# andyljones/megastep

Hardware: AMD Instinct MI355X
Metric: env-steps/sec (higher is better)
Workload: dtype f32

## Files before the change

include/megastep_hip.h:

```cpp
#ifndef MEGASTEP_HIP_H
#define MEGASTEP_HIP_H

#ifdef __cplusplus
extern "C" {
#endif

#define MS_ABI_VERSION 17

#define MS_OK            0
#define MS_EINVAL       -1
#define MS_EHIP         -2
#define MS_EUNSUPPORTED -3
#define MS_ENODEVICE    -4

typedef struct MsConfig {
    float agent_radius;
    int   res;
    float fov;
    float fps;
} MsConfig;

typedef struct MsScenery {
    int n_envs, n_agents, n_model;
    const float* lights_vals;
    const int*   lights_widths;
    const int*   lights_starts;
    float*       lines_vals;
    const int*   lines_widths;
    const int*   lines_starts;
    const int*   lines_inverse;
    const float* textures_vals;
    const int*   textures_widths;
    const int*   textures_starts;
    const int*   textures_inverse;
    const float* model;
    float*       baked_vals;
    int n_lines_total, n_lights_total, n_texels_total;
    unsigned*    lg_vals;
    const int*   lg_starts;
    const float* lg_geom;
    float        lg_cell;
    int          lg_max_cells;
    unsigned*    lg_list;
    unsigned*    lg_pool;
    int          lg_pool_size;
    float*       lg_pool_rows;
    const int*   env_geom;
    unsigned long long* bake_vis;
    const long long*    bake_vis_starts;
    long long           bake_vis_words;
    const unsigned*       wg_cells;
    const int*            wg_starts;
    const float*          wg_geom;
    float                 wg_cell;
    float                 wg_reach_lo, wg_reach;
    float                 wg_near;
    const unsigned*       wg_pool;
    const long long*      wg_pool_base;
    const float*          wg_near_rows;
    float model_radius;
} MsScenery;

typedef struct MsAgents {
    float* angles;
    float* positions;
    float* angvelocity;
    float* velocity;
    float* headings;
} MsAgents;

typedef struct MsRender {
    int*   indices;
    float* locations;
    float* dots;
    float* distances;
    float* screen;
    int*   workspace;
    float* obs_rgb;
    float* obs_depth;
    int    obs_subsample;
    float  obs_max_depth;
    int*   obs_centre;
    int*       seen_stamp;
    const int* seen_epoch;
    int*       seen_count;
} MsRender;

#define MS_RENDER_WORKSPACE_INTS(N, A, R) (18 + (long long)(N)*(A)*(((R) + 63)/64) + 2*(long long)(N)*(A))

int         ms_abi_version(void);
const char* ms_strerror(int code);
int         ms_last_hip_error(void);
int         ms_device_count(void);

int ms_bake(const MsScenery* scenery, const MsConfig* config, void* hip_stream);

typedef struct MsMovement {
    const long long* actions;
    const float*     table;
    int              n_actions;
    float            keep;
} MsMovement;

typedef struct MsStepExtras {
    unsigned char*   respawn_mask;
    const long long* respawn_choice;
    const float*     spawn_positions;
    const float*     spawn_angles;
    int              n_spawns;
    int              respawn_after;
    int*             lifespans;
    int*             max_lifespans;
    const int*       fresh_max;
    float*           imu;
    float            imu_ang_scale, imu_speed_scale;
} MsStepExtras;

int ms_move_physics(const MsScenery* scenery, const MsAgents* agents, const MsMovement* movement ,
                    float* progress, const MsConfig* config, void* hip_stream);
int ms_physics(const MsScenery* scenery, const MsAgents* agents, float* progress,
               const MsConfig* config, void* hip_stream);
int ms_step_physics(const MsScenery* scenery, const MsAgents* agents, const MsMovement* movement, const MsStepExtras* extras,
                    float* progress, const MsConfig* config, void* hip_stream);

int ms_render(const MsScenery* scenery, const MsAgents* agents, const MsRender* out,
              const MsConfig* config, void* hip_stream);

int ms_step_render(const MsScenery* scenery, const MsAgents* agents, float* progress, const MsRender* out,
                   const MsConfig* config, void* hip_stream);
int ms_move_step_render(const MsScenery* scenery, const MsAgents* agents, const MsMovement* movement, const MsStepExtras* extras,
                        float* progress, const MsRender* out, const MsConfig* config, void* hip_stream);

typedef struct MsDeathmatch {
    const int*      centre;
    const float*    positions;
    const float*    upper;
    float           clearance, hit_damage, tick_damage;
    float*          health;
    float*          damage;
    unsigned char*  dead;
    unsigned char*  reset_out;
    float*          reward;
    float*          health_obs;
    unsigned char*  matchings;
} MsDeathmatch;
int ms_deathmatch_shoot(int n_envs, int n_agents, const MsDeathmatch* dm, void* hip_stream);

typedef struct MsExplorer {
    int*            tally;
    int*            before;
    int*            lengths;
// ... 85 lines not shown
```

megastep_amd/_lib.py:

```python
import ctypes as C
import os
import subprocess
import torch

_HERE = os.path.dirname(os.path.abspath(__file__))
CSRC = os.path.join(_HERE, 'csrc')
LIB_PATH = os.environ.get('MEGASTEP_HIP_LIB') or os.path.join(CSRC, 'libmegastep_hip.so')
ABI_VERSION = 17

_f32p = C.POINTER(C.c_float)
_i32p = C.POINTER(C.c_int)


class MsConfig(C.Structure):
    _fields_ = [('agent_radius', C.c_float), ('res', C.c_int), ('fov', C.c_float), ('fps', C.c_float)]


class MsScenery(C.Structure):
    _fields_ = [
        ('n_envs', C.c_int), ('n_agents', C.c_int), ('n_model', C.c_int),
        ('lights_vals', C.c_void_p), ('lights_widths', C.c_void_p), ('lights_starts', C.c_void_p),
        ('lines_vals', C.c_void_p), ('lines_widths', C.c_void_p), ('lines_starts', C.c_void_p),
        ('lines_inverse', C.c_void_p),
        ('textures_vals', C.c_void_p), ('textures_widths', C.c_void_p), ('textures_starts', C.c_void_p),
        ('textures_inverse', C.c_void_p),
        ('model', C.c_void_p), ('baked_vals', C.c_void_p),
        ('n_lines_total', C.c_int), ('n_lights_total', C.c_int), ('n_texels_total', C.c_int),
        ('lg_vals', C.c_void_p), ('lg_starts', C.c_void_p), ('lg_geom', C.c_void_p), ('lg_cell', C.c_float),
        ('lg_max_cells', C.c_int), ('lg_list', C.c_void_p), ('lg_pool', C.c_void_p), ('lg_pool_size', C.c_int), ('lg_pool_rows', C.c_void_p),
        ('env_geom', C.c_void_p), ('bake_vis', C.c_void_p), ('bake_vis_starts', C.c_void_p), ('bake_vis_words', C.c_longlong),
        ('wg_cells', C.c_void_p), ('wg_starts', C.c_void_p), ('wg_geom', C.c_void_p), ('wg_cell', C.c_float),
        ('wg_reach_lo', C.c_float), ('wg_reach', C.c_float), ('wg_near', C.c_float), ('wg_pool', C.c_void_p), ('wg_pool_base', C.c_void_p), ('wg_near_rows', C.c_void_p),
        ('model_radius', C.c_float)]


class MsWallGridParent(C.Structure):
    _fields_ = [('cells', C.c_void_p), ('starts', C.c_void_p), ('geom', C.c_void_p), ('cell', C.c_float), ('pool', C.c_void_p)]


class MsAgents(C.Structure):
    _fields_ = [('angles', C.c_void_p), ('positions', C.c_void_p), ('angvelocity', C.c_void_p), ('velocity', C.c_void_p),
                ('headings', C.c_void_p)]


class MsMovement(C.Structure):
    _fields_ = [('actions', C.c_void_p), ('table', C.c_void_p), ('n_actions', C.c_int), ('keep', C.c_float)]


class MsStepExtras(C.Structure):
    _fields_ = [('respawn_mask', C.c_void_p), ('respawn_choice', C.c_void_p), ('spawn_positions', C.c_void_p),
                ('spawn_angles', C.c_void_p), ('n_spawns', C.c_int), ('respawn_after', C.c_int),
                ('lifespans', C.c_void_p), ('max_lifespans', C.c_void_p), ('fresh_max', C.c_void_p),
                ('imu', C.c_void_p), ('imu_ang_scale', C.c_float), ('imu_speed_scale', C.c_float)]


class MsRender(C.Structure):
    _fields_ = [('indices', C.c_void_p), ('locations', C.c_void_p), ('dots', C.c_void_p), ('distances', C.c_void_p),
                ('screen', C.c_void_p), ('workspace', C.c_void_p), ('obs_rgb', C.c_void_p), ('obs_depth', C.c_void_p),
                ('obs_subsample', C.c_int), ('obs_max_depth', C.c_float), ('obs_centre', C.c_void_p),
                ('seen_stamp', C.c_void_p), ('seen_epoch', C.c_void_p), ('seen_count', C.c_void_p)]


class MsDeathmatch(C.Structure):
    _fields_ = [('centre', C.c_void_p), ('positions', C.c_void_p), ('upper', C.c_void_p), ('clearance', C.c_float), ('hit_damage', C.c_float),
                ('tick_damage', C.c_float), ('health', C.c_void_p), ('damage', C.c_void_p), ('dead', C.c_void_p), ('reset_out', C.c_void_p),
                ('reward', C.c_void_p), ('health_obs', C.c_void_p), ('matchings', C.c_void_p)]


class MsExplorer(C.Structure):
    _fields_ = [('tally', C.c_void_p), ('before', C.c_void_p), ('lengths', C.c_void_p), ('epoch', C.c_void_p), ('over', C.c_void_p),
                ('slack', C.c_int), ('pixels', C.c_int), ('reset_out', C.c_void_p), ('reward', C.c_void_p), ('potential', C.c_void_p),
                ('length_out', C.c_void_p)]


class MsRaycast(C.Structure):
    _fields_ = [('n_rays', C.c_int), ('origins', C.c_void_p), ('dirs', C.c_void_p), ('near_plane', C.c_float),
                ('indices', C.c_void_p), ('locations', C.c_void_p), ('dots', C.c_void_p), ('distances', C.c_void_p),
                ('agents', C.c_void_p), ('grid_rays', C.c_void_p)]


class MsOverhead(C.Structure):
    _fields_ = [('n_images', C.c_int), ('n_views', C.c_int), ('height', C.c_int), ('width', C.c_int), ('envs', C.c_void_p),
                ('views', C.c_void_p), ('half_width', C.c_float), ('lit', C.c_int), ('background', C.c_float*3),
                ('rgb', C.c_void_p), ('indices', C.c_void_p)]


class MsNavGrid(C.Structure):
    _fields_ = [('n_envs', C.c_int), ('cell', C.c_float), ('clearance', C.c_float), ('geom', C.c_void_p), ('starts', C.c_void_p),
                ('max_framed', C.c_int), ('free_cells', C.c_void_p)]


class MsNavFields(C.Structure):
    _fields_ = [('n_goals', C.c_int), ('goals', C.c_void_p), ('mask', C.c_void_p), ('fields', C.c_void_p), ('passes', C.c_void_p)]


class MsNavQuery(C.Structure):
    _fields_ = [('n_points', C.c_int), ('points', C.c_void_p), ('goal', C.c_void_p), ('fields', C.c_void_p), ('n_goals', C.c_int),
                ('out', C.c_void_p)]


SYMBOLS = ('ms_host_ray_interval_wide', 'ms_debug_ray_groups', 'ms_debug_last_render_groups', 'ms_debug_last_step_fused', 'ms_step_render', 'ms_move_step_render', 'ms_debug_ray_group_tail', 'ms_debug_physics_pack', 'ms_host_render_plan', 'ms_host_render_block', 'ms_host_physics_pack', 'ms_debug_pair_telemetry', 'ms_test_arithmetic', 'ms_abi_version', 'ms_strerror', 'ms_last_hip_error', 'ms_device_count', 'ms_bake', 'ms_physics', 'ms_move_physics',
           'ms_step_physics', 'ms_deathmatch_shoot', 'ms_explorer_books',
           'ms_render', 'ms_raycast', 'ms_camera_rays', 'ms_overhead', 'ms_nav_free', 'ms_nav_fields', 'ms_nav_query', 'ms_debug_overhead_cull', 'ms_host_overhead_keeps', 'ms_host_sincospi', 'ms_host_bake_point_bin', 'ms_host_bake_wall_bins',
           'ms_wallgrid_scan', 'ms_wallgrid_fill', 'ms_host_wall_hidden', 'ms_host_wall_sectors', 'ms_host_wallgrid_cell', 'ms_host_wall_arc',
           'ms_host_wedge_meets', 'ms_host_agents_apart', 'ms_host_wall_beyond_reach', 'ms_host_ray_interval', 'ms_host_fold_hits', 'ms_host_lightgrid_cell', 'ms_host_wall_reach')


def _source_hash():
    import hashlib
    h = hashlib.sha256()
    import glob
    for path in (os.path.join(CSRC, 'megastep_hip.hip'), *sorted(glob.glob(os.path.join(CSRC, 'kernels', '*.h'))),
                 os.path.join(_HERE, '..', 'include', 'megastep_hip.h'), os.path.join(_HERE, '..', 'include', 'megastep_hip_test.h'),
                 os.path.join(CSRC, 'Makefile')):
        with open(path, 'rb') as f:
            h.update(f.read())
    return h.hexdigest()


def build(force=False):
    import fcntl
    stamp = LIB_PATH + '.srchash'
    want = _source_hash()

    def fresh():
        return os.path.exists(LIB_PATH) and os.path.exists(stamp) and open(stamp).read().strip() == want

    if force or not fresh():
        with open(os.path.join(CSRC, '.build.lock'), 'w') as lock:
            fcntl.flock(lock, fcntl.LOCK_EX)
            if force or not fresh():
                import shutil
                hipcc = os.environ.get('HIPCC', '/opt/rocm/bin/hipcc')
                if shutil.which('make') is None or shutil.which(hipcc) is None or not os.access(CSRC, os.W_OK):
                    raise NoToolchain(f'no make / {hipcc} on this host, or {CSRC} is read-only')
                proc = subprocess.run(['make', '-C', CSRC, '-B', 'libmegastep_hip.so'], capture_output=True, text=True)
                if proc.returncode != 0:
                    raise RuntimeError(f'hipcc build of libmegastep_hip.so failed:\n{proc.stdout}\n{proc.stderr}')
    return LIB_PATH


class NoToolchain(OSError):
    """The library cannot be rebuilt here for want of tools (not because its sources do not compile)."""


_lib = None


def lib():
    global _lib
    if _lib is None:
        if not os.environ.get('MEGASTEP_HIP_LIB'):
            try:
                build()
            except NoToolchain as e:
                if not os.path.exists(LIB_PATH):
                    raise
                import warnings
                warnings.warn(f'{LIB_PATH} could not be rebuilt from the sources next to it ({e}); loading it as it is')
        handle = C.CDLL(LIB_PATH)
        missing = [s for s in SYMBOLS if not hasattr(handle, s)]
        if missing:
            raise ImportError(f'{LIB_PATH} does not export {missing}')
        handle.ms_abi_version.restype = C.c_int
        handle.ms_strerror.restype = C.c_char_p
        handle.ms_strerror.argtypes = [C.c_int]
        handle.ms_last_hip_error.restype = C.c_int
        handle.ms_device_count.restype = C.c_int
        handle.ms_bake.argtypes = [C.POINTER(MsScenery), C.POINTER(MsConfig), C.c_void_p]
        handle.ms_physics.argtypes = [C.POINTER(MsScenery), C.POINTER(MsAgents), C.c_void_p, C.POINTER(MsConfig), C.c_void_p]
        handle.ms_move_physics.argtypes = [C.POINTER(MsScenery), C.POINTER(MsAgents), C.POINTER(MsMovement), C.c_void_p,
                                           C.POINTER(MsConfig), C.c_void_p]
        handle.ms_step_physics.argtypes = [C.POINTER(MsScenery), C.POINTER(MsAgents), C.POINTER(MsMovement), C.POINTER(MsStepExtras),
                                           C.c_void_p, C.POINTER(MsConfig), C.c_void_p]
        handle.ms_step_render.argtypes = [C.POINTER(MsScenery), C.POINTER(MsAgents), C.c_void_p, C.POINTER(MsRender), C.POINTER(MsConfig), C.c_void_p]
        handle.ms_step_render.restype = C.c_int
        handle.ms_move_step_render.argtypes = [C.POINTER(MsScenery), C.POINTER(MsAgents), C.POINTER(MsMovement), C.POINTER(MsStepExtras),
                                               C.c_void_p, C.POINTER(MsRender), C.POINTER(MsConfig), C.c_void_p]
        handle.ms_move_step_render.restype = C.c_int
        handle.ms_debug_last_step_fused.argtypes = []
        handle.ms_debug_last_step_fused.restype = C.c_int
        handle.ms_explorer_books.argtypes = [C.c_int, C.POINTER(MsExplorer), C.c_void_p]
        handle.ms_explorer_books.restype = C.c_int
        handle.ms_deathmatch_shoot.argtypes = [C.c_int, C.c_int, C.POINTER(MsDeathmatch), C.c_void_p]
        handle.ms_deathmatch_shoot.restype = C.c_int
        handle.ms_render.argtypes = [C.POINTER(MsScenery), C.POINTER(MsAgents), C.POINTER(MsRender), C.POINTER(MsConfig), C.c_void_p]
        handle.ms_raycast.argtypes = [C.POINTER(MsScenery), C.POINTER(MsAgents), C.POINTER(MsRaycast), C.POINTER(MsConfig), C.c_void_p]
        handle.ms_camera_rays.argtypes = [C.POINTER(MsAgents), C.c_int, C.c_int, C.POINTER(MsConfig), C.c_void_p, C.c_void_p]
        handle.ms_overhead.argtypes = [C.POINTER(MsScenery), C.POINTER(MsAgents), C.POINTER(MsOverhead), C.c_void_p]
        handle.ms_nav_free.argtypes = [C.POINTER(MsScenery), C.POINTER(MsNavGrid), C.c_void_p]
        handle.ms_nav_fields.argtypes = [C.POINTER(MsNavGrid), C.POINTER(MsNavFields), C.c_void_p]
        handle.ms_nav_query.argtypes = [C.POINTER(MsNavGrid), C.POINTER(MsNavQuery), C.c_void_p]
        handle.ms_debug_overhead_cull.argtypes = [C.c_int]
        handle.ms_debug_overhead_cull.restype = C.c_int
        handle.ms_host_overhead_keeps.argtypes = [_f32p, C.c_int, C.c_int, C.c_int, C.c_int, C.c_float, _f32p]
        handle.ms_host_overhead_keeps.restype = C.c_int
        handle.ms_host_sincospi.argtypes = [C.c_float, _f32p, _f32p]
        handle.ms_host_bake_point_bin.argtypes = [C.c_float]*4
        handle.ms_host_bake_point_bin.restype = C.c_int
        handle.ms_host_bake_wall_bins.argtypes = [C.c_float]*6 + [_i32p, _i32p]
        handle.ms_host_bake_wall_bins.restype = None
        handle.ms_wallgrid_scan.argtypes = [C.POINTER(MsScenery), C.POINTER(MsWallGridParent), C.c_void_p, C.c_int, C.c_int, C.c_void_p,
                                            C.c_void_p, C.c_void_p, C.c_void_p]
        handle.ms_wallgrid_fill.argtypes = [C.POINTER(MsScenery), C.c_void_p, C.c_int, C.c_int, C.c_void_p, C.c_void_p, C.c_void_p,
                                            C.c_void_p, C.c_void_p, C.c_void_p]
        handle.ms_host_wall_sectors.argtypes = [C.c_float]*4 + [_f32p, _i32p, _i32p, _f32p, _i32p]
        handle.ms_host_wall_sectors.restype = None
        handle.ms_host_wall_arc.argtypes = [C.c_float]*4 + [_f32p, _i32p, _i32p]
        handle.ms_host_wall_arc.restype = None
        handle.ms_host_wedge_meets.argtypes = [C.c_float]*4 + [C.c_int, C.c_int]
        handle.ms_host_wedge_meets.restype = C.c_int
        handle.ms_host_ray_interval.argtypes = [_f32p, _f32p, C.c_int, C.c_float, C.c_float, C.c_int, _i32p, _i32p]
        handle.ms_host_ray_interval.restype = None
        handle.ms_host_ray_interval_wide.argtypes = [_f32p, _f32p, C.c_int, C.c_float, C.c_float, C.c_int, C.c_int, _i32p, _i32p]
        handle.ms_host_ray_interval_wide.restype = None
        handle.ms_debug_ray_groups.argtypes = [C.c_int]
        handle.ms_debug_ray_groups.restype = C.c_int
        handle.ms_debug_last_render_groups.argtypes = []
        handle.ms_debug_last_render_groups.restype = C.c_int
        handle.ms_debug_ray_group_tail.argtypes = [C.c_float, C.c_int]
        handle.ms_debug_physics_pack.argtypes = [C.c_int]
        handle.ms_debug_physics_pack.restype = C.c_int
        handle.ms_host_render_plan.argtypes = [C.c_int, C.c_int, C.c_int, C.c_int, C.c_int, C.c_float, C.c_int, C.POINTER(C.c_int)]
        handle.ms_host_render_plan.restype = C.c_longlong
        handle.ms_host_render_block.argtypes = [C.c_int, C.c_int, C.c_int, C.c_int, C.c_int, C.c_float, C.c_int, C.c_longlong, C.POINTER(C.c_int)]
        handle.ms_host_render_block.restype = C.c_int
        handle.ms_host_physics_pack.argtypes = [C.c_int, C.c_int, C.c_int, C.c_int]
        handle.ms_host_physics_pack.restype = C.c_int
        handle.ms_debug_ray_group_tail.restype = C.c_int
        handle.ms_debug_pair_telemetry.argtypes = [C.c_int]
        handle.ms_debug_pair_telemetry.restype = C.c_int
        handle.ms_test_arithmetic.argtypes = [C.c_void_p]*7 + [C.c_longlong, C.c_void_p]
        handle.ms_test_arithmetic.restype = C.c_int
        handle.ms_host_fold_hits.argtypes = [_f32p, _i32p, C.c_int, _i32p, _f32p, _i32p]
        handle.ms_host_fold_hits.restype = C.c_int
        handle.ms_host_lightgrid_cell.argtypes = [C.c_void_p, C.c_int, C.c_void_p, C.c_int, C.c_float, C.c_float, C.c_int, C.c_int, C.c_float,
                                                  C.c_int, C.c_void_p, C.c_void_p, C.c_int]
        handle.ms_host_lightgrid_cell.restype = C.c_int
        handle.ms_host_agents_apart.argtypes = [_f32p, _f32p, C.c_float]
        handle.ms_host_agents_apart.restype = C.c_int
        handle.ms_host_wall_beyond_reach.argtypes = [_f32p, _f32p, C.c_float]
        handle.ms_host_wall_beyond_reach.restype = C.c_int
        handle.ms_host_wall_reach.argtypes = [_f32p, C.c_float]
        handle.ms_host_wall_reach.restype = C.c_float
        handle.ms_host_wall_hidden.argtypes = [C.c_float]*4 + [_f32p, _f32p, C.c_float]
        handle.ms_host_wall_hidden.restype = C.c_int
        handle.ms_host_wallgrid_cell.argtypes = [C.c_void_p, C.c_int, C.c_float, C.c_float, C.c_int, C.c_int, C.c_float, C.c_int,
                                                 C.c_float, C.c_float, C.c_float, C.c_void_p, C.c_void_p]
        handle.ms_host_wallgrid_cell.restype = None
        for name in ('ms_bake', 'ms_physics', 'ms_move_physics', 'ms_step_physics', 'ms_render', 'ms_raycast', 'ms_camera_rays', 'ms_overhead', 'ms_nav_free', 'ms_nav_fields', 'ms_nav_query', 'ms_wallgrid_scan', 'ms_wallgrid_fill'):
            getattr(handle, name).restype = C.c_int
        if handle.ms_abi_version() != ABI_VERSION:
            raise ImportError(f'{LIB_PATH} has ABI {handle.ms_abi_version()}, this package needs {ABI_VERSION}; rebuild it')
        _lib = handle
    return _lib


def check(code):
    if code != 0:
        h = lib()
        raise RuntimeError(f'megastep_hip: {h.ms_strerror(code).decode()} (code {code}, hipError {h.ms_last_hip_error()})')


_raw_stream = getattr(torch._C, '_cuda_getCurrentRawStream', None)


def _stream(dev):
    if _raw_stream is not None and dev.index is not None:
        return C.c_void_p(_raw_stream(dev.index))
    return C.c_void_p(torch.cuda.current_stream(dev).cuda_stream)


class _on:

    def __init__(self, dev):
        self._guard = None if dev.index == torch.cuda.current_device() else torch.cuda.device(dev)

    def __enter__(self):
        if self._guard is not None:
            self._guard.__enter__()

    def __exit__(self, *exc):
        if self._guard is not None:
            self._guard.__exit__(*exc)
```

megastep_amd/csrc/kernels/lighting.h:

```cpp
__device__ inline bool light_blocked(P2 I, P2 U, float ax, float ay, float vx, float vy) {
    const P2 V = p2(vx, vy);
    const float UxV = cross(U, V);
    const float ad = fabsf(UxV);
    if (ad < 1.e-3f) return false;
    const P2 PQ = p2(ax, ay) - I;
    const uint32_t sg = f_bits(UxV) & 0x80000000u;
    const float nt = bits_f(f_bits(cross(PQ, U)) ^ sg);
    const float cs = cross(PQ, V);
    const float ns = bits_f(f_bits(cs) ^ sg);
    if (!((nt > 0.f) & (nt < ad) & (ns > 0.f))) return false;
    return div_inrange(cs, UxV) < .999f;
}

struct LightPair { float ax, ay, vx, vy, ix, iy; int light; int pad; };
constexpr int LG_PAIRS = 64;

struct LightScene {
    int n_agents, n_model;
    const float* lights_vals; const int* lights_widths; const int* lights_starts;
    const unsigned* lg_vals; const int* lg_starts; const float* lg_geom; float lg_cell;
    const unsigned* lg_list; const unsigned* lg_pool; const float4* lg_pool_rows;
    unsigned by_m_mul, by_m_sh1, by_m_sh2;
};

__device__ inline float grid_light_intensity(
        const LightScene sc, const MsAgents& ag, const int n, const int lane, const bool dynamic, const int nearest_idx,
        const float cx_l, const float cy_l, const int L, const float4* __restrict__ ln,
        LightPair* s_pair, unsigned* s_shadow, unsigned& telemetry, [[maybe_unused]] unsigned* clk = nullptr) {
#if MS_PROBE
#define LG_CLK(k, v) { asm volatile("" :: "v"(v)); clk[k] = (unsigned)clock64(); }
#else
#define LG_CLK(k, v)
#endif
    const int A = sc.n_agents, AF = sc.n_agents*sc.n_model;
    const int n_lights = sc.lights_widths[n];
    const bool MANY = n_lights > WAVE;
    float acc_in = AMBIENT;
    for (int first_light = 0; ; first_light += WAVE) {
    const int ni = min(WAVE, n_lights - first_light);
    const float* __restrict__ lights = sc.lights_vals + 3*((size_t)sc.lights_starts[n] + first_light);
    const float4 geom = reinterpret_cast<const float4*>(sc.lg_geom)[n];
    float Ix = 0.f, Iy = 0.f, Ii = 0.f;
    if (lane < ni) { Ix = lights[3*lane]; Iy = lights[3*lane + 1]; Ii = lights[3*lane + 2]; }
    int my_target = -1;
    if (dynamic) {
        const unsigned t_ = __umulhi(sc.by_m_mul, (unsigned)nearest_idx);
        my_target = (int)((t_ + (((unsigned)nearest_idx - t_) >> sc.by_m_sh1)) >> sc.by_m_sh2);
    }

    uint4 st = make_uint4(0u, 0u, 0u, 0u);
    uint2 lst = make_uint2(0u, 0u);
    if (!MANY) {
        const float fx = floorf((cx_l - geom.x)/sc.lg_cell), fy = floorf((cy_l - geom.y)/sc.lg_cell);
        const bool inside = dynamic & (fx >= 0.f) & (fx < geom.z) & (fy >= 0.f) & (fy < geom.w);
        const size_t cell_id = (size_t)sc.lg_starts[n] + (inside ? (int)fy*(int)geom.z + (int)fx : 0);
        const uint4 st_ = reinterpret_cast<const uint4*>(sc.lg_vals)[cell_id];
        uint2 lst_ = make_uint2(0u, 0u);
        if (sc.lg_list) lst_ = reinterpret_cast<const uint2*>(sc.lg_list)[cell_id];
        st.x = inside ? st_.x : 0u; st.y = inside ? st_.y : 0u; st.z = inside ? st_.z : 0u; st.w = inside ? st_.w : 0u;
        lst.x = inside ? lst_.x : 0u; lst.y = inside ? lst_.y : 0u;
    }
    LG_CLK(0, st.x + __float_as_uint(Ii))
    const bool shortcut = !MANY && __ballot((lane < ni) & !(Ii >= 0.f)) == 0ull;
    const bool light_ok = ((Ii == 0.f) || ((Ii >= 1.e-12f) && (Ii <= 1.e12f))) && (fabsf(Ix) <= 1.e6f) && (fabsf(Iy) <= 1.e6f);
    const bool point_ok = (fabsf(cx_l) <= 1.e6f) && (fabsf(cy_l) <= 1.e6f);
    const bool nice = __ballot(((lane < ni) && !light_ok) || (dynamic && !point_ok)) == 0ull;
    auto contribution = [&](const float num, const float den) { return nice ? div_inrange(num, den) : num/den; };
    float part = AMBIENT;
    for (unsigned long long rem = MANY ? 0ull : __ballot(dynamic); rem; ) {
        const int j = __ffsll((long long)rem) - 1;
        const unsigned sw[4] = {(unsigned)__builtin_amdgcn_readlane((int)st.x, j), (unsigned)__builtin_amdgcn_readlane((int)st.y, j),
                                (unsigned)__builtin_amdgcn_readlane((int)st.z, j), (unsigned)__builtin_amdgcn_readlane((int)st.w, j)};
        const bool same = dynamic & (st.x == sw[0]) & (st.y == sw[1]) & (st.z == sw[2]) & (st.w == sw[3]);
        rem &= ~__ballot(same);
        #pragma unroll
        for (int k = 0; k < 4; k++) {
            for (unsigned lw = sw[k] & ~(sw[k] >> 1) & 0x55555555u; lw; lw &= lw - 1) {
                const int i = 16*k + ((__ffs((int)lw) - 1) >> 1);
                const float d2 = len2(p2(readlane_f(Ix, i), readlane_f(Iy, i)) - p2(cx_l, cy_l));
                if (same) part += contribution(LUMINANCE*readlane_f(Ii, i), ms_max(d2, 1.f));
            }
        }
    }
    bool has_unk = false;
    {
        const unsigned wd[4] = {st.x, st.y, st.z, st.w};
        #pragma unroll
        for (int k = 0; k < 4; k++) {
            const int nv = min(max(ni - 16*k, 0), 16);
            const unsigned valid = (nv == 16) ? 0x55555555u : (((1u << (2*nv)) - 1u) & 0x55555555u);
            has_unk |= (~(wd[k] | (wd[k] >> 1)) & valid) != 0u;
        }
    }
    LG_CLK(1, part)
    const bool saturated = dynamic & shortcut & (part >= 1.001f);
    const bool need = dynamic & !saturated & has_unk;
    if (!__ballot(need)) return MANY ? acc_in : (saturated ? 1.f : ms_min(part, 1.f));
    telemetry = 0x80000000u | (unsigned)__popcll(__ballot(need)) | ((unsigned)min(ni, 63) << 25);

    auto status = [&](int i) {
        const unsigned wd = (i < 16) ? st.x : (i < 32) ? st.y : (i < 48) ? st.z : st.w;
        return (wd >> (2*(i & 15))) & 3u;
    };
    unsigned long long shadow = 0ull;
    const bool sweep = need & (lst.y == 0u);
    const int n_cd = (need & !sweep) ? (int)(lst.y & 0x7fffffffu) : 0;
    telemetry |= (unsigned)__popcll(__ballot(sweep)) << 7;
    if (__ballot(n_cd > 0)) {
        s_shadow[2*lane] = 0u; s_shadow[2*lane + 1] = 0u;
// ... 153 lines not shown
```

megastep_amd/csrc/kernels/overhead.h:

```cpp
constexpr int OV_TILE = 16;
constexpr int OV_CHUNK = 1024;
static_assert(OV_TILE*OV_TILE == WG, "one pixel per lane");
static_assert(OV_CHUNK % WG == 0 && OV_CHUNK >= 2*WG, "a window of WG lines must fit after a partly filled list");

struct OvArgs {
    const int* envs;
    const float* views;
    float* rgb;
    int* indices;
    long long block0;
    int n_views, height, width, tiles_x, tiles_y;
    float half_width, h2;
    float bg_r, bg_g, bg_b;
    int lit, with_agents, cull;
};

struct OvBox { float x0, y0, x1, y1, mag; bool finite; };

__host__ __device__ inline OvBox ov_footprint(const float g0, const float g1, const float g2, const float g3, const float g4,
                                              const float g5, const int i0, const int j0, const int i1, const int j1) {
    const float ua = (float)j0 + .5f, ub = (float)j1 + .5f, wa = (float)i0 + .5f, wb = (float)i1 + .5f;
    const float xs[4] = {(g0*ua + g1*wa) + g2, (g0*ub + g1*wa) + g2, (g0*ua + g1*wb) + g2, (g0*ub + g1*wb) + g2};
    const float ys[4] = {(g3*ua + g4*wa) + g5, (g3*ub + g4*wa) + g5, (g3*ua + g4*wb) + g5, (g3*ub + g4*wb) + g5};
    OvBox b{xs[0], ys[0], xs[0], ys[0], 0.f, true};
    for (int c = 0; c < 4; c++) {
        b.finite = b.finite && isfinite(xs[c]) && isfinite(ys[c]);
        b.x0 = fminf(b.x0, xs[c]); b.x1 = fmaxf(b.x1, xs[c]);
        b.y0 = fminf(b.y0, ys[c]); b.y1 = fmaxf(b.y1, ys[c]);
    }
    const float sx = 1e-5f*((fabsf(g0)*ub + fabsf(g1)*wb) + fabsf(g2));
    const float sy = 1e-5f*((fabsf(g3)*ub + fabsf(g4)*wb) + fabsf(g5));
    b.finite = b.finite && isfinite(sx) && isfinite(sy);
    b.x0 -= sx; b.x1 += sx; b.y0 -= sy; b.y1 += sy;
    b.mag = fmaxf(fmaxf(fabsf(b.x0), fabsf(b.x1)), fmaxf(fabsf(b.y0), fabsf(b.y1)));
    return b;
}

__host__ __device__ inline bool ov_keeps(const OvBox& b, const float h, const float4 L) {
    if (!b.finite) return true;
    const float mag = fmaxf(fmaxf(fabsf(L.x), fabsf(L.y)), fmaxf(fabsf(L.z), fabsf(L.w)));
    const float r = h + 1e-5f*(h + mag + b.mag);
    const float x0 = b.x0 - r, x1 = b.x1 + r, y0 = b.y0 - r, y1 = b.y1 + r;
    if ((fmaxf(L.x, L.z) < x0) || (fminf(L.x, L.z) > x1) || (fmaxf(L.y, L.w) < y0) || (fminf(L.y, L.w) > y1)) return false;
    const float vx = L.z - L.x, vy = L.w - L.y;
    const float cx = .5f*(x0 + x1), cy = .5f*(y0 + y1), ex = .5f*(x1 - x0), ey = .5f*(y1 - y0);
    const float qx = cx - L.x, qy = cy - L.y;
    const float sep = fabsf(vx*qy - vy*qx);
    const float reach = ex*fabsf(vy) + ey*fabsf(vx);
    const float tol = 1e-5f*(fabsf(vx) + fabsf(vy))*(fabsf(qx) + fabsf(qy) + ex + ey + fabsf(vx) + fabsf(vy));
    return !(sep > reach + tol);
}

struct OvBest { float d2; int idx; float t; };

__device__ inline void ov_fold(const float x, const float y, const float4 L, const int l, const float h2, OvBest& b) {
    const float vx = L.z - L.x, vy = L.w - L.y, px = x - L.x, py = y - L.y;
    const float vv = vx*vx + vy*vy;
    float t = vv > 0.f ? (px*vx + py*vy)/vv : 0.f;
    t = t < 0.f ? 0.f : (t > 1.f ? 1.f : t);
    const float dx = px - t*vx, dy = py - t*vy;
    const float d2 = dx*dx + dy*dy;
    if ((d2 <= h2) & ((d2 < b.d2) | ((d2 == b.d2) & (l < b.idx)))) { b.d2 = d2; b.idx = l; b.t = t; }
}

__global__ __launch_bounds__(WG) void overhead_kernel(const MsScenery sc, const MsAgents ag, const OvArgs a) {
    __shared__ float4 s_rows[OV_CHUNK];
    __shared__ int s_idx[OV_CHUNK];
    __shared__ int s_wave[WAVES];
    const int tid = threadIdx.x, lane = tid % WAVE, wave = tid / WAVE;
    const long long blk = a.block0 + blockIdx.x;
    const int tiles = a.tiles_x*a.tiles_y;
    const long long kv = blk / tiles;
    const int tile = (int)(blk - kv*tiles);
    const int k = (int)(kv / a.n_views);
    const int ty = tile / a.tiles_x, tx = tile - ty*a.tiles_x;
    const int i0 = ty*OV_TILE, j0 = tx*OV_TILE;
    const int i = i0 + tid / OV_TILE, j = j0 + tid % OV_TILE;
    const bool live = (i < a.height) & (j < a.width);
    const long long hw = (long long)a.height*a.width;
    const long long at = kv*hw + (long long)i*a.width + j;
    const int e = __builtin_amdgcn_readfirstlane(a.envs ? a.envs[k] : k);

    OvBest best{INFINITY, INT_MAX, 0.f};
    int base = 0, AF = 0;
    if ((e >= 0) & (e < sc.n_envs)) {
        const float* const g = a.views + kv*6;
        const float g0 = g[0], g1 = g[1], g2 = g[2], g3 = g[3], g4 = g[4], g5 = g[5];
        const float u = (float)j + .5f, w = (float)i + .5f;
        const float x = (g0*u + g1*w) + g2, y = (g3*u + g4*w) + g5;
        const OvBox box = ov_footprint(g0, g1, g2, g3, g4, g5, i0, j0, min(i0 + OV_TILE - 1, a.height - 1),
                                       min(j0 + OV_TILE - 1, a.width - 1));
        const int L = sc.lines_widths[e];
        base = sc.lines_starts[e];
        const int A = sc.n_agents, M = sc.n_model;
        AF = A*M;
        const float4* const rows = reinterpret_cast<const float4*>(sc.lines_vals) + base;
        int count = 0;
        for (int l0 = 0; l0 < L; l0 += WG) {
            const int l = l0 + tid;
            bool keep = false;
            float4 row = make_float4(0.f, 0.f, 0.f, 0.f);
            if (l < L) {
                if (a.with_agents && l < AF) {
                    const int agent = l / M;
                    float s, c;
                    sincospi_f(ag.angles[e*A + agent]/180.f, s, c);
                    const float2 p = reinterpret_cast<const float2*>(ag.positions)[e*A + agent];
                    row = drawn_row(s, c, p.x, p.y, reinterpret_cast<const float4*>(sc.model)[l - agent*M]);
                } else {
                    row = rows[l];
                }
                keep = !a.cull || ov_keeps(box, a.half_width, row);
            }
            const unsigned long long m = __ballot(keep);
            if (lane == 0) s_wave[wave] = (int)__popcll(m);
            __syncthreads();
            int off = count, total = 0;
            for (int q = 0; q < WAVES; q++) {
                const int c = s_wave[q];
                off += q < wave ? c : 0;
                total += c;
            }
            off += (int)__popcll(m & ((1ull << lane) - 1ull));
            if (keep) { s_rows[off] = row; s_idx[off] = l; }
            count += total;
            __syncthreads();
            if (count > OV_CHUNK - WG || l0 + WG >= L) {
                for (int q = 0; q < count; q++) ov_fold(x, y, s_rows[q], s_idx[q], a.h2, best);
                count = 0;
                __syncthreads();
            }
        }
    }

    if (!live) return;
    float r = a.bg_r, gr = a.bg_g, bl = a.bg_b;
    int idx = -1;
    if (best.idx != INT_MAX) {
        idx = best.idx;
        r = gr = bl = 0.f;
        const int gl = base + idx;
        const int tw = a.rgb ? sc.textures_widths[gl] : 0;
        if (tw > 0) {
            const int q = min((int)(best.t*(float)tw), tw - 1);
            const long long tex = (long long)sc.textures_starts[gl] + q;
            r = sc.textures_vals[3*tex]; gr = sc.textures_vals[3*tex + 1]; bl = sc.textures_vals[3*tex + 2];
            if (a.lit && idx >= AF) {
                const float bk = sc.baked_vals[tex];
// ... 11 lines not shown
```

megastep_amd/csrc/kernels/physics.h:

```cpp
constexpr int PHYS_AHEAD = 4;
constexpr int PHYS_FEW = 4;
constexpr int PHYS_PAIRS = (PHYS_FEW + 1)*WAVE;

__device__ inline void spawn_pose(const MsStepExtras& ex, const int i, float2& p, float& ang) {
    const long long c = min(max(ex.respawn_choice[i], 0ll), (long long)ex.n_spawns - 1);
    p = reinterpret_cast<const float2*>(ex.spawn_positions)[(size_t)i*ex.n_spawns + c];
    ang = ex.spawn_angles[(size_t)i*ex.n_spawns + c];
}
__device__ inline int lifespan_tick(const MsStepExtras& ex, const int i, bool& reset) {
    const int life = ex.lifespans[i] + 1;
    reset = reset | (life >= ex.max_lifespans[i]);
    return reset ? 0 : life;
}
__device__ inline void move_velocity(const float keep, const float ang, const float dx, const float dy, const float dw, float2& v, float& w) {
    const float a_ = 0.017453292519943295f*ang;
    const float s_ = sinf(a_), c_ = cosf(a_);
    const float gx = c_*dx - s_*dy, gy = s_*dx + c_*dy;
    if (keep == 0.f) { w = dw; v = make_float2(gx, gy); }
    else { w = keep*w + dw; v = make_float2(keep*v.x + gx, keep*v.y + gy); }
}
__device__ inline int near_count(const uint4 hdr, const float reach, const float reach_lo) {
    return (int)((reach <= reach_lo) ? (hdr.w & 0xffffu) : (hdr.w >> 16));
}
__device__ inline bool integrate(const float x, const float fps, float2& p, float& ang, float2& v, float& w) {
    p.x = p.x + x*v.x/fps;
    p.y = p.y + x*v.y/fps;
    ang = normalize_degrees(ang + x*w/fps);
    const bool stopped = x < 1;
    if (stopped) { v = make_float2(0.f, 0.f); w = 0.f; }
    return stopped;
}
__device__ inline float3 imu_reading(const MsStepExtras& ex, const float ang, const float2 v, const float w) {
    const float a_ = 0.017453292519943295f*ang;
    const float s_ = sinf(a_), c_ = cosf(a_);
    return make_float3(w*ex.imu_ang_scale, (c_*v.x + s_*v.y)*ex.imu_speed_scale, (-s_*v.x + c_*v.y)*ex.imu_speed_scale);
}

template <int MOVE, int EXTRA, int PACK = 0>
__global__ __launch_bounds__(WAVE) void physics_kernel(
        const MsScenery sc, const MsAgents ag, float* __restrict__ progress,
        const float agent_radius, const float fps, const MsMovement mv, const MsStepExtras ex, const int pack_envs, const Divisor by_a) {
    PROBE_INIT
    extern __shared__ float4 s_dyn[];
    __shared__ float4 s_wall[PHYS_PAIRS];
    __shared__ int s_tag[PHYS_PAIRS];
    const int A1 = sc.n_agents, AF = sc.n_agents*sc.n_model;
    const int lane = threadIdx.x;
    const int n = PACK ? blockIdx.x*pack_envs : blockIdx.x;
    const int E = PACK ? min(pack_envs, sc.n_envs - n) : 1;
    const int A = PACK ? A1*E : A1;
    const int nA = n*A1;
    [[maybe_unused]] const int lane_env = PACK ? min(div_by(lane, by_a), E - 1) : 0;
    float4* s_task = s_dyn;
    float4* s_box = s_task + A;
    float* s_reach2 = reinterpret_cast<float*>(s_box + A);
    unsigned* s_prog = reinterpret_cast<unsigned*>(s_reach2 + A);
    const float2* pos2 = reinterpret_cast<const float2*>(ag.positions);
    const float2* vel2 = reinterpret_cast<const float2*>(ag.velocity);

    const int L = sc.lines_widths[n];
    const float4* __restrict__ ln = reinterpret_cast<const float4*>(sc.lines_vals) + sc.lines_starts[n];
    const LineRows rows(ln, L);
    const bool gridded = sc.wg_cells != nullptr;
    const float4 wg_geom_n = reinterpret_cast<const float4*>(sc.wg_geom)[n + lane_env];
    const int wg_start_n = sc.wg_starts[n + lane_env];
    float4 w[PHYS_AHEAD];
    #pragma unroll
    for (int k = 0; k < PHYS_AHEAD; k++) w[k] = make_float4(0.f, 0.f, 0.f, 0.f);
    if (!gridded) {
        #pragma unroll
        for (int k = 0; k < PHYS_AHEAD; k++) w[k] = rows.chunk(lane, AF + k*WAVE);
    }
    float2 my_p, my_v;
    float my_w, my_ang;
    my_p = make_float2(0.f, 0.f); my_v = make_float2(0.f, 0.f); my_w = 0.f; my_ang = 0.f;
    if (lane < A) { my_p = pos2[nA + lane]; my_v = vel2[nA + lane]; my_w = ag.angvelocity[nA + lane]; my_ang = ag.angles[nA + lane]; }

    if constexpr (EXTRA == 1) {
        for (int t = lane; t < A; t += WAVE) {
            const int i = nA + t;
            bool reset = ex.respawn_mask && ex.respawn_mask[i];
            if (ex.lifespans) {
                ex.lifespans[i] = lifespan_tick(ex, i, reset);
                if (reset) ex.max_lifespans[i] = ex.fresh_max[i];
                if (ex.respawn_mask) ex.respawn_mask[i] = reset ? 1 : 0;
            }
            if (reset && ex.spawn_positions && !ex.respawn_after) {
                float2 p; float ang;
                spawn_pose(ex, i, p, ang);
                if (t == lane) { my_p = p; my_ang = ang; my_v = make_float2(0.f, 0.f); my_w = 0.f; }
                reinterpret_cast<float2*>(ag.positions)[i] = p;
                ag.angles[i] = ang;
                reinterpret_cast<float2*>(ag.velocity)[i] = make_float2(0.f, 0.f);
                ag.angvelocity[i] = 0.f;
            }
        }
    }
    if constexpr (MOVE == 1) {
        const bool small_table = 3*mv.n_actions <= WAVE;
        const float tab = mv.table[min(lane, 3*mv.n_actions - 1)];
        auto moved = [&](const int i, const float ang, float2& v, float& w, const float dx, const float dy, const float dw) {
            move_velocity(mv.keep, ang, dx, dy, dw, v, w);
            ag.angvelocity[i] = w;
            reinterpret_cast<float2*>(ag.velocity)[i] = v;
        };
        {
            const long long act = min(max(mv.actions[nA + min(lane, A - 1)], 0ll), (long long)mv.n_actions - 1);
            float dx, dy, dw;
            if (small_table) { dx = __shfl(tab, 3*(int)act, WAVE); dy = __shfl(tab, 3*(int)act + 1, WAVE); dw = __shfl(tab, 3*(int)act + 2, WAVE); }
            else { dx = mv.table[3*act]; dy = mv.table[3*act + 1]; dw = mv.table[3*act + 2]; }
            if (lane < A) moved(nA + lane, my_ang, my_v, my_w, dx, dy, dw);
        }
        for (int t = lane + WAVE; t < A; t += WAVE) {
            float2 v = vel2[nA + t];
            float w = ag.angvelocity[nA + t];
            const long long act = min(max(mv.actions[nA + t], 0ll), (long long)mv.n_actions - 1);
            moved(nA + t, ag.angles[nA + t], v, w, mv.table[3*act], mv.table[3*act + 1], mv.table[3*act + 2]);
        }
    }
    float4 my_box = make_float4(INFINITY, INFINITY, -INFINITY, -INFINITY);
    float my_reach = 0.f;
    for (int t = lane; t < A; t += WAVE) {
        const float2 pp = (t == lane) ? my_p : pos2[nA + t], mm = (t == lane) ? my_v : vel2[nA + t];
        const P2 p0 = p2(pp.x, pp.y);
        const P2 v0 = p2(mm.x, mm.y)/fps;
        const float reach = wall_reach(p0, v0, agent_radius);
        s_reach2[t] = reach_squared(reach);
        const float4 box = make_float4(p0.x - reach, p0.y - reach, p0.x + reach, p0.y + reach);
        if (t == lane) { my_box = box; my_reach = (reach == reach) ? reach : INFINITY; }
        s_box[t] = box;
        s_task[t] = make_float4(p0.x, p0.y, v0.x, v0.y);
// ... 200 lines not shown
```

megastep_amd/csrc/kernels/raycast.h:

```cpp

struct RayFold { float s; int idx; float t, vx, vy; };

__device__ inline void ray_fold(const P2 p, const P2 ru, const float near_s, const float4 L, const int l, RayFold& f) {
    const P2 v = p2(L.z - L.x, L.w - L.y);
    const P2 pq = p2(L.x, L.y) - p;
    const float d = cross(ru, v), nt = cross(pq, ru);
    const float ad = fabsf(d);
    const float ntp = __uint_as_float(__float_as_uint(nt) ^ (__float_as_uint(d) & 0x80000000u));
    if ((ad >= 1.e-3f) & (ntp <= ad) & (ntp >= -1e-30f*ad)) {
        const Isect q = intersect(p, ru, p2(L.x, L.y), v);
        const bool hit = (0 <= q.t) & (q.t <= 1);
        const bool better = (near_s < q.s) & (q.s < f.s - 1.e-4f);
        if (hit & better) { f.s = q.s; f.idx = l; f.t = q.t; f.vx = v.x; f.vy = v.y; }
    }
}

__global__ __launch_bounds__(WG) void raycast_kernel(const MsScenery sc, const MsAgents ag, const MsRaycast q, const int with_agents,
                                                     const int gridded, const int n_total) {
    const int i_raw = blockIdx.x*WG + threadIdx.x;
    const bool live = i_raw < n_total;
    const int i = live ? i_raw : n_total - 1;
    const int n = i / q.n_rays;
    const float2 o = reinterpret_cast<const float2*>(q.origins)[i];
    const float2 d = reinterpret_cast<const float2*>(q.dirs)[i];
    const P2 p = p2(o.x, o.y), ru = p2(d.x, d.y);
    const float rlen = len(ru);
    const float near_s = q.near_plane/rlen;
    const int A = sc.n_agents, M = sc.n_model, AF = A*M;
    RayFold f{INFINITY, -1, NAN, 0.f, 0.f};
    auto fold_agents = [&](const int e) {
        for (int a = 0; a < A; a++) {
            float s, c;
            sincospi_f(ag.angles[e*A + a]/180.f, s, c);
            const float2 pa = reinterpret_cast<const float2*>(ag.positions)[e*A + a];
            for (int m = 0; m < M; m++)
                ray_fold(p, ru, near_s, drawn_row(s, c, pa.x, pa.y, reinterpret_cast<const float4*>(sc.model)[m]), a*M + m, f);
        }
    };
    const int n_w = __builtin_amdgcn_readfirstlane(n);
    const bool one_env = __ballot(n != n_w) == 0ull;

    if (one_env) {
        const int L = sc.lines_widths[n_w];
        const float4* const rows = reinterpret_cast<const float4*>(sc.lines_vals) + sc.lines_starts[n_w];
        if (with_agents) fold_agents(n_w);
        bool listed = false;
        int cell = -1;
        if (gridded) {
            bool inside;
            const int c = wg_cell_at(reinterpret_cast<const float4*>(sc.wg_geom)[n_w], sc.wg_cell, p.x, p.y, inside);
            const float ru2 = len2(ru);
            listed = inside & (ru2 >= 1.f) & (ru2 <= WG_MAX_RU2);
            cell = listed ? sc.wg_starts[n_w] + c : -1;
        }
        unsigned long long pending = __ballot(listed);
        int walk = 0;
        for (unsigned long long todo = pending; todo && walk <= L - AF;) {
            const int cell_w = __builtin_amdgcn_readlane(cell, __ffsll((long long)todo) - 1);
            walk += (int)reinterpret_cast<const uint4*>(sc.wg_cells)[cell_w].y;
            todo &= ~__ballot(cell == cell_w);
        }
        if (walk > L - AF) pending = 0ull;
        bool done = false;
        while (pending) {
            const int cell_w = __builtin_amdgcn_readlane(cell, __ffsll((long long)pending) - 1);
            const uint4 hdr = reinterpret_cast<const uint4*>(sc.wg_cells)[cell_w];
            const int count = (int)hdr.y;
            const bool mine = cell == cell_w;
            pending &= ~__ballot(mine);
            if (mine) {
                int wa8, wb8;
                const float pa = pseudo_angle(ru.x, ru.y);
                wg_wedge(pa, pa, wa8, wb8);
                const unsigned* const vis = sc.wg_pool + sc.wg_pool_base[n_w] + hdr.x;
                for (int k = 0; k < count; k++) {
                    const unsigned e = vis[k];
                    const int l = AF + (int)(e & 0xffffu);
                    if (wg_arcs_meet((int)((e >> 16) & 255u), (int)(e >> 24), wa8, wb8) & (l < L)) ray_fold(p, ru, near_s, rows[l], l, f);
                }
                done = true;
            }
        }
        if (__ballot(!done))
            for (int l = AF; l < L; l++) {
                const float4 row = rows[l];
                if (!done) ray_fold(p, ru, near_s, row, l, f);
            }
        if (q.grid_rays) {
            const unsigned long long took = __ballot(live & done);
            if (took && (int)threadIdx.x % WAVE == __ffsll((long long)__ballot(1)) - 1) atomicAdd(q.grid_rays, (int)__popcll(took));
        }
    } else {
        const int L = sc.lines_widths[n];
        const float4* const rows = reinterpret_cast<const float4*>(sc.lines_vals) + sc.lines_starts[n];
        if (with_agents) fold_agents(n);
        for (int l = AF; l < L; l++) ray_fold(p, ru, near_s, rows[l], l, f);
    }

    if (!live) return;
    float dt = NAN;
// ... 24 lines not shown
```

megastep_amd/csrc/kernels/render.h:

```cpp
constexpr int PAIRS = 128;

struct Cand { float pqx, pqy, vx, vy; };

__device__ __attribute__((noinline)) float2 sincospi_called(const float x) {
    float s_, c_;
    sincospi_f(x, s_, c_);
    return make_float2(s_, c_);
}

__device__ inline float4 drawn_row(const float s, const float c, const float px, const float py, const float4 mdl) {
    float4 w;
    w.x = c*mdl.x - s*mdl.y + px; w.y = s*mdl.x + c*mdl.y + py;
    w.z = c*mdl.z - s*mdl.w + px; w.w = s*mdl.z + c*mdl.w + py;
    return w;
}
__device__ inline void camera_ray(const float cs, const float sn, const int r, const float Rf, const float half_screen,
                                  const float inv_res, float& rx, float& ry) {
    const float num = (Rf - 2*(float)r - 1)*half_screen;
    const float uy = inv_res != 0.f ? num*inv_res : div_inrange(num, Rf);
    rx = cs*1.f - sn*uy; ry = sn*1.f + cs*uy;
}
__host__ inline float camera_inv_res(const int R, const float half_screen) {
    return ((R & (R - 1)) == 0 && half_screen > 1e-3f) ? 1.f/(float)R : 0.f;
}

__device__ __attribute__((noinline)) float4 drawn_line_of(const float* angles, const float* positions, const float* model,
                                                          const int n_agents, const int M, const int n, const int l) {
    const int a = l / M, m = l - a*M;
    float s, c;
    sincospi_f(angles[n*n_agents + a]/180.f, s, c);
    const float2 p = reinterpret_cast<const float2*>(positions)[n*n_agents + a];
    return drawn_row(s, c, p.x, p.y, reinterpret_cast<const float4*>(model)[m]);
}
__device__ inline float4 drawn_line(const MsScenery& sc, const MsAgents& ag, int n, int l) {
    return drawn_line_of(ag.angles, ag.positions, sc.model, sc.n_agents, sc.n_model, n, l);
}

struct Filt { int l, r; float lw, rw; };
__device__ inline Filt tex_filter(float x, int w) {
    Filt f;
    const float y = ms_min(x*(w + 1), (float)(w - 1));
    f.l = (int)ms_max(y - 1, 0.f);
    f.r = (int)ms_min(y, (float)(w - 1));
    const float ld = fabsf(y - (f.l + 1)) + 1.e-3f;
    const float rd = fabsf(y - (f.r + 1)) + 1.e-3f;
    const float den = ld + rd, r_den = rcp_refined(den);
    f.lw = div_by_refined(rd, den, r_den);
    f.rw = div_by_refined(ld, den, r_den);
    return f;
}

__device__ inline float sqrt_normal(const float x) {
    const float s = __builtin_amdgcn_sqrtf(x);
    const float dn = bits_f(f_bits(s) - 1u), up = bits_f(f_bits(s) + 1u);
    const float r_dn = __builtin_fmaf(-dn, s, x), r_up = __builtin_fmaf(-up, s, x);
    float r = (r_dn <= 0.f) ? dn : s;
    r = (r_up > 0.f) ? up : r;
    return r;
}

__device__ __attribute__((noinline)) float sqrtf_called(const float x) { return sqrtf(x); }
__device__ inline float sqrt_any(const float x) {
    float r = sqrt_normal(x);
    if (__builtin_expect(!(x >= 1.e-30f) && x != 0.f, 0) || __builtin_expect(!(x <= 1.e30f), 0)) r = sqrtf_called(x);
    return r;
}

struct RenderConsts {
    float x_clip, c_b;
    Divisor by_f, by_g, by_m;
    Divisor by_f1, by_g1;
    int envs_lo, envs_rem, tail;
    int skip_own;
    float inv_res;
    int telemetry;
    int ws_headings;
};
struct RenderConstsStep : RenderConsts {
    float* progress;
    float fps;
    const unsigned* wg_cells_physics;
    MsMovement mv;
    MsStepExtras ex;
};
enum { OUT_INDICES = 1, OUT_LOCATIONS = 2, OUT_DOTS = 4, OUT_DISTANCES = 8, OUT_SCREEN = 16, OUT_RGB = 32, OUT_DEPTH = 64, OUT_CENTRE = 128,
       OUT_SEEN = 256 };
__global__ __launch_bounds__(WG) void arithmetic_test_kernel(const float* __restrict__ n, const float* __restrict__ d, float* __restrict__ q_inrange,
                                                             float* __restrict__ q_ieee, const float* __restrict__ x, float* __restrict__ r_any,
                                                             float* __restrict__ r_ieee, const long long count) {
    const long long i = (long long)blockIdx.x*WG + threadIdx.x;
    if (i >= count) return;
    if (q_inrange) q_inrange[i] = div_by_refined(n[i], d[i], rcp_refined(d[i]));
    if (q_ieee) q_ieee[i] = n[i]/d[i];
    if (r_any) r_any[i] = sqrt_any(x[i]);
    if (r_ieee) r_ieee[i] = sqrtf(x[i]);
}

__host__ __device__ inline bool render_block(const int b, const int n_blocks, const int A, const int R, const int ng, const RenderConsts& rc,
                                             int& n, int& a, int& r0, int& span, int& fan) {
    const int xcd = b & 7, ix = b >> 3;
    fan = b;
    if (ng == 1) {
        const int q8 = n_blocks >> 3, r8 = n_blocks & 7;
        fan = xcd*q8 + (xcd < r8 ? xcd : r8) + ix;
        const int G = (R + WAVE - 1)/WAVE, F = A*G;
        n = div_by(fan, rc.by_f); const int rem = fan - n*F; a = div_by(rem, rc.by_g); r0 = (rem - a*G)*WAVE; span = WAVE;
        return true;
    }
    const int NR = ng*WAVE;
    const int e_x = rc.envs_lo + (xcd < rc.envs_rem ? 1 : 0), first_x = xcd*rc.envs_lo + (xcd < rc.envs_rem ? xcd : rc.envs_rem);
    const int t_x = rc.tail < e_x ? rc.tail : e_x;
    const int Gw = (R + NR - 1)/NR, w_x = (e_x - t_x)*A*Gw;
    const bool single = ix >= w_x;
    const int f = single ? ix - w_x : ix;
    const int G = single ? (R + WAVE - 1)/WAVE : Gw, F = A*G;
    const Divisor df = Divisor{single ? rc.by_f1.mul : rc.by_f.mul, single ? rc.by_f1.sh1 : rc.by_f.sh1, single ? rc.by_f1.sh2 : rc.by_f.sh2};
    const Divisor dg = Divisor{single ? rc.by_g1.mul : rc.by_g.mul, single ? rc.by_g1.sh1 : rc.by_g.sh1, single ? rc.by_g1.sh2 : rc.by_g.sh2};
    const int nn = div_by(f, df), rem = f - nn*F;
    if (nn >= (single ? t_x : e_x - t_x)) return false;
    a = div_by(rem, dg);
    n = first_x + (single ? e_x - t_x : 0) + nn;
    span = single ? WAVE : NR;
    r0 = (rem - a*G)*span;
    return true;
}

__global__ __launch_bounds__(WG) void render_prep_kernel(const MsAgents ag, int* __restrict__ workspace,
                                                         const int n_agents_total, const int headings_at) {
    const int i = blockIdx.x*WG + threadIdx.x;
    if (i == 0) { workspace[0] = 0; workspace[1] = 0; workspace[2] = 0; workspace[3] = 0; workspace[4] = 0; }
    if (i < n_agents_total) {
        float s, c;
        sincospi_f(ag.angles[i]/180.f, s, c);
        reinterpret_cast<float2*>(workspace + headings_at)[i] = make_float2(s, c);
    }
}


struct RenderArgs { MsScenery sc; MsAgents ag; MsRender out; float agent_radius, half_screen; int R, n_fans; RenderConsts rc; };
static_assert(offsetof(RenderArgs, ag) == sizeof(MsScenery) && offsetof(RenderArgs, n_fans) + 4 == offsetof(RenderArgs, rc),
              "RenderArgs must mirror render_kernel's parameters");
typedef const RenderArgs __attribute__((address_space(4)))* LateArgs;
__device__ inline LateArgs late_args() {
    LateArgs p = (LateArgs)__builtin_amdgcn_kernarg_segment_ptr();
    asm volatile("" : "+s"(p));
    return p;
}

__host__ inline uint32_t host_f_bits(const float f) { uint32_t u; memcpy(&u, &f, 4); return u; }
__host__ inline float host_bits_f(const uint32_t u) { float f; memcpy(&f, &u, 4); return f; }
__host__ inline unsigned long long slot_min(unsigned long long* slot, const unsigned long long key) {
    const unsigned long long old = *slot;
    if (key < old) *slot = key;
    return old;
}
__host__ inline unsigned long long hit_key(const float sv, const int line) { return ((unsigned long long)host_f_bits(sv) << 32) | (unsigned)line; }
__host__ inline bool hit_loser_matters(const unsigned long long key, const float sv, const unsigned long long old, unsigned long long& lose1) {
    const unsigned oh = (unsigned)(old >> 32);
    if (oh == 0xffffffffu) return false;
    const bool won = key < old;
    const float so = host_bits_f(oh);
    const float front = won ? sv : so, back = won ? so : sv;
    lose1 = won ? old : key;
    return back < front + 4.e-4f;
}
__host__ inline bool hit_resolve(const unsigned long long best, const unsigned long long second, const unsigned long long third,
                                 float& nearest_s, int& nearest_idx) {
    bool ambiguous = false;
    if (best != ~0ull) {
        const float s1 = host_bits_f((uint32_t)(best >> 32)), s2 = host_bits_f((uint32_t)(second >> 32)), s3 = host_bits_f((uint32_t)(third >> 32));
        const int i1 = (int)(uint32_t)best, i2 = (int)(uint32_t)second;
        nearest_s = s1;
        nearest_idx = i1;
        if ((second != ~0ull) && !(s1 < s2 - 1.e-4f)) {
            if ((third == ~0ull) || (s2 < s3 - 1.e-4f)) {
                const bool first_is_1 = i1 < i2;
                const float sa = first_is_1 ? s1 : s2, sb = first_is_1 ? s2 : s1;
                const int ia = first_is_1 ? i1 : i2, ib = first_is_1 ? i2 : i1;
                const bool b_wins = sb < sa - 1.e-4f;
                nearest_s = b_wins ? sb : sa;
                nearest_idx = b_wins ? ib : ia;
            } else {
                ambiguous = true;
            }
        }
    }
    return ambiguous;
}

__host__ __device__ inline float rcp_approx(const float x) {
#if defined(__HIP_DEVICE_COMPILE__)
    return __builtin_amdgcn_rcpf(x);
#else
    return 1.f/x;
#endif
}
__host__ __device__ inline void agent_frame(const float cs, const float sn, const float pqx, const float pqy, const float dbx, const float dby,
                                            float& xa, float& ya, float& xb, float& yb) {
    xa = __builtin_fmaf(cs, pqx, sn*pqy); ya = __builtin_fmaf(cs, pqy, -(sn*pqx));
    xb = __builtin_fmaf(cs, dbx, sn*dby); yb = __builtin_fmaf(cs, dby, -(sn*dbx));
}
__host__ __device__ inline void ray_interval(float xa, float ya, float xb, float yb, const bool live, const float x_clip,
                                    const float c_a, const float c_b, const float g0, const float last_local, int& lo, int& len,
                                    const float n_rays = 64.f) {
    const bool fa = xa >= x_clip, fb = xb >= x_clip;
    const bool inc = fa | fb;
    const float ia = fa ? ya*rcp_approx(xa) : 0.f, ib = fb ? yb*rcp_approx(xb) : 0.f;
    const float fra = __builtin_fmaf(-ia, c_b, c_a), frb = __builtin_fmaf(-ib, c_b, c_a);
    const float marg = __builtin_fmaf(1e-4f, fabsf(fra) + fabsf(frb), 0.05f);
    const float edge = (xa*yb - ya*xb > 0.f) ? -INFINITY : INFINITY;
    const float ra = fa ? fra : -edge, rb = fb ? frb : edge;
    const float flo = fminf(fmaxf(fminf(ra, rb) - (marg + g0), 0.f), n_rays);
    const float fhi = fmaxf(fminf(fmaxf(ra, rb) + (marg - g0), last_local), -1.f);
    lo = (int)ceilf(flo);
    const int n_ = (int)floorf(fhi) - lo + 1;
    len = (live & inc) ? (n_ > 0 ? n_ : 0) : 0;
}

#ifndef MS_WAVES
#define MS_WAVES 6
#endif
#ifndef MS_AHEAD
#define MS_AHEAD 1
#endif
#ifndef MS_VCAP
#define MS_VCAP 128
#endif
#ifndef MS_VCAP_WIDE
#define MS_VCAP_WIDE 110
#endif
#ifndef MS_WAVES_WIDE
#define MS_WAVES_WIDE 6
#endif
template <int OBS, int SHADE = 1, int NG = 1, int STEP = 0>
__global__ __launch_bounds__(WAVE) __attribute__((amdgpu_waves_per_eu(NG > 1 ? MS_WAVES_WIDE : MS_WAVES, NG > 1 ? MS_WAVES_WIDE : MS_WAVES))) void render_kernel(
        const MsScenery sc, const MsAgents ag, const MsRender out,
        const float agent_radius, const float half_screen, const int R, const int n_fans,
        const std::conditional_t<STEP == 1, RenderConstsStep, RenderConsts> rc) {
    static_assert(STEP == 0 || NG == 1, "the fused step: one group of rays");
    PROBE_INIT
    static_assert(NG == 1 || NG == 2 || NG == 4, "one, two or four ray groups per wave");
    [[maybe_unused]] constexpr int NR = WAVE*NG;
    constexpr int VCAP = NG == 1 ? MS_VCAP : MS_VCAP_WIDE;
    constexpr int O_EPI = NG > 1 ? 24*VCAP + 256 : 0;
    constexpr int LDS_PER_WAVE = NG == 1 ? 24*VCAP + 3072 : O_EPI + 2816 + 6*VCAP;
    __shared__ __attribute__((aligned(16))) unsigned char s_raw[LDS_PER_WAVE];

    int lane = threadIdx.x;
#define LANE_AFRESH asm volatile("" : "+v"(lane))
    Cand* const s_cand_w = reinterpret_cast<Cand*>(&s_raw[0]);
    float* const s_screen_w = reinterpret_cast<float*>(&s_raw[O_EPI]);

    const int b = blockIdx.x;
    [[maybe_unused]] int fan = b;
    const int A = sc.n_agents, AF = sc.n_agents*sc.n_model;
    int n, a, r0, span;
    if (!render_block(b, n_fans, A, R, NG, rc, n, a, r0, span, fan)) return;
    const int r = r0 + lane;
    const int r_last = min(r0 + span - 1, R - 1);
    [[maybe_unused]] const int n_live = r_last - r0 + 1;

    const int L = sc.lines_widths[n];
    const int base = sc.lines_starts[n];
    const float4 wg_geom_n = reinterpret_cast<const float4*>(sc.wg_geom)[n];
    const int wg_start_n = sc.wg_starts[n];
    const long long wg_pool_base_n = sc.wg_pool_base[n];
    float4* __restrict__ ln = reinterpret_cast<float4*>(sc.lines_vals) + base;
    const LineRows rows(ln, L);
    float ag_s = 0.f, ag_c = 0.f;
    float2 ag_p = make_float2(0.f, 0.f);
    auto load_agents = [&]() {
    ag_s = 0.f; ag_c = 0.f; ag_p = make_float2(0.f, 0.f);
    const int lane_a = n*A + min(lane, A - 1);
    if (ag.headings) {
        const float4 h = reinterpret_cast<const float4*>(ag.headings)[lane_a];
        const float angle = ag.angles[lane_a];
        const float2 p_ = reinterpret_cast<const float2*>(ag.positions)[lane_a];
        if (lane < A) {
            ag_s = h.y; ag_c = h.z; ag_p = p_;
            if (f_bits(h.x) != f_bits(angle)) { const float2 sc_ = sincospi_called(angle/180.f); ag_s = sc_.x; ag_c = sc_.y; }
        }
    } else if (lane < A) {
        if (out.workspace) {
            const float2 sc_ = reinterpret_cast<const float2*>(out.workspace + rc.ws_headings)[n*A + lane];
            ag_s = sc_.x; ag_c = sc_.y;
        } else {
            const float2 sc_ = sincospi_called(ag.angles[n*A + lane]/180.f);
            ag_s = sc_.x; ag_c = sc_.y;
        }
        ag_p = reinterpret_cast<const float2*>(ag.positions)[n*A + lane];
    }
    };
    if constexpr (STEP == 1) {
        float2 p_ = reinterpret_cast<const float2*>(ag.positions)[n], v_ = reinterpret_cast<const float2*>(ag.velocity)[n];
        float w_ = ag.angvelocity[n], ang_ = ag.angles[n];
        const MsStepExtras& ex = rc.ex;
        bool respawn_now = false;
        float2 spawn_p = make_float2(0.f, 0.f);
        float spawn_ang = 0.f;
        if (ex.respawn_mask || ex.lifespans) {
            bool reset = ex.respawn_mask && ex.respawn_mask[n];
            if (ex.lifespans) {
                const int life = lifespan_tick(ex, n, reset);
                const int fresh = ex.fresh_max[n];
                __builtin_amdgcn_wave_barrier();
                if (lane == 0) {
                    if (reset) ex.max_lifespans[n] = fresh;
                    ex.lifespans[n] = life;
                    if (ex.respawn_mask) ex.respawn_mask[n] = reset ? 1 : 0;
                }
            }
            if (reset && ex.spawn_positions) {
                spawn_pose(ex, n, spawn_p, spawn_ang);
                respawn_now = true;
                if (!ex.respawn_after) {
                    p_ = spawn_p; ang_ = spawn_ang; v_ = make_float2(0.f, 0.f); w_ = 0.f;
                    if (lane == 0) {
                        reinterpret_cast<float2*>(ag.positions)[n] = p_;
                        ag.angles[n] = ang_;
                        reinterpret_cast<float2*>(ag.velocity)[n] = v_;
                        ag.angvelocity[n] = 0.f;
                    }
                }
            }
        }
        if (rc.mv.actions) {
            const long long act = min(max(rc.mv.actions[n], 0ll), (long long)rc.mv.n_actions - 1);
            move_velocity(rc.mv.keep, ang_, rc.mv.table[3*act], rc.mv.table[3*act + 1], rc.mv.table[3*act + 2], v_, w_);
            if (lane == 0) {
                ag.angvelocity[n] = w_;
                reinterpret_cast<float2*>(ag.velocity)[n] = v_;
            }
        }
        const P2 p0 = p2(p_.x, p_.y);
        const P2 v0 = p2(v_.x, v_.y)/rc.fps;
        const float reach = wall_reach(p0, v0, agent_radius);
        const float reach2 = reach_squared(reach);
        const float my_reach = (reach == reach) ? reach : INFINITY;
        const float4 tk = make_float4(p0.x, p0.y, v0.x, v0.y);
        bool listed_p = false;
// ... 39 lines not shown
            }
            rc.progress[n] = x;
        }
        if (ex.imu) {
            const float3 m = imu_reading(ex, ang_, v_, w_);
            if (lane == 0) {
                ex.imu[3*n] = m.x;
                ex.imu[3*n + 1] = m.y;
                ex.imu[3*n + 2] = m.z;
            }
        }
        ag_s = hsc.x; ag_c = hsc.y; ag_p = p_;
    } else {
        load_agents();
    }
    constexpr int AHEAD = MS_AHEAD;

    const float4 mdl_draw = reinterpret_cast<const float4*>(sc.model)[min(lane, sc.n_model - 1)];
    const float4 mdl_first = reinterpret_cast<const float4*>(sc.model)[lane - div_by(lane, rc.by_m)*sc.n_model];
    auto agent_line_m = [&](const int l_, const bool have_row, const float4 row) {
        const int l = min(max(l_, 0), AF - 1);
        if (A > WAVE) return drawn_line(sc, ag, n, l);
        const int la = div_by(l, rc.by_m);
        const float s_ = __shfl(ag_s, la, WAVE), c_ = __shfl(ag_c, la, WAVE);
        const float px_ = __shfl(ag_p.x, la, WAVE), py_ = __shfl(ag_p.y, la, WAVE);
        float4 mdl = row;
        if (!have_row) mdl = reinterpret_cast<const float4*>(sc.model)[l - la*sc.n_model];
        return drawn_row(s_, c_, px_, py_, mdl);
    };
    auto agent_line = [&](const int l_) { return agent_line_m(l_, false, make_float4(0.f, 0.f, 0.f, 0.f)); };
    float sn, cs;
    float2 pp;
    if (A <= WAVE) {
        sn = readlane_f(ag_s, a); cs = readlane_f(ag_c, a);
        pp = make_float2(readlane_f(ag_p.x, a), readlane_f(ag_p.y, a));
    } else {
        const float2 sc_ = sincospi_called(ag.angles[n*A + a]/180.f);
        sn = sc_.x; cs = sc_.y;
        pp = reinterpret_cast<const float2*>(ag.positions)[n*A + a];
    }
    PROBE_AT(1, pp.x)
    unsigned wg_first = 0u;
    int wg_count = -1;
    if (sc.wg_cells) {
        bool inside;
        const int cell_id = __builtin_amdgcn_readfirstlane(wg_start_n + wg_cell_at(wg_geom_n, sc.wg_cell, pp.x, pp.y, inside));
        const uint4 hdr = reinterpret_cast<const uint4*>(sc.wg_cells)[cell_id];
        wg_first = inside ? hdr.x : 0u;
        wg_count = inside ? (int)hdr.y : -1;
        if constexpr (NG > 1) {
            wg_first = (unsigned)__builtin_amdgcn_readfirstlane((int)wg_first);
            wg_count = __builtin_amdgcn_readfirstlane(wg_count);
        }
    }
    if (r0 == 0) {
        for (int m0 = 0; m0 < sc.n_model; m0 += WAVE) {
            const float4 w = agent_line_m(a*sc.n_model + m0 + lane, m0 == 0, mdl_draw);
            if (m0 + lane < sc.n_model) ln[a*sc.n_model + m0 + lane] = w;
        }
    }
    const float Rf = (float)R;
    auto ray_len = [&](const float rx_, const float ry_) {
        return sqrt_normal(rx_*rx_ + ry_*ry_);
    };
    auto ray_of = [&](const int r_, float& rx_, float& ry_, float& rlen_, float& near_) {
        camera_ray(cs, sn, r_, Rf, half_screen, rc.inv_res, rx_, ry_);
        rlen_ = ray_len(rx_, ry_);
        near_ = div_inrange(agent_radius, rlen_);
    };
    float rx, ry, rlen, near;
    ray_of(r, rx, ry, rlen, near);

    const float c_a = 0.5f*(Rf - 1.f), c_b = rc.c_b;
    const float x_clip = rc.x_clip;
    const float g0 = (float)r0;

    constexpr bool COLOUR = SHADE != 0;
    static_assert(COLOUR || OBS == 1, "without colour `screen` is NULL: the OBS instantiation");
    static_assert(OBS != 2 || (COLOUR && STEP == 0), "no per-ray planes at all: a colour instantiation");
    constexpr bool PLANES = OBS != 2;
    constexpr bool MASKED = !COLOUR || (OBS >= 1 && NG == 1);
    [[maybe_unused]] const int out_mask_ = MASKED ? (out.obs_subsample >> 8) : 0;
#define MS_WANTED(BIT, PTR) (MASKED ? ((out_mask_ & (BIT)) != 0) : ((PTR) != nullptr))
    auto winner_of = [&](const int nearest_idx, float4& hw_mem, int& tex_w, int& tstart) {
        const LateArgs late = late_args();
        const bool want_texel_row = COLOUR || (OBS && MS_WANTED(OUT_SEEN, late->out.seen_stamp));
        const bool want_line = want_texel_row || MS_WANTED(OUT_LOCATIONS, late->out.locations) || MS_WANTED(OUT_DOTS, late->out.dots);
        const int row = min(max(nearest_idx, 0), max(L - 1, 0));
        hw_mem = make_float4(0.f, 0.f, 0.f, 0.f); tex_w = 1; tstart = 0;
        if (want_line) hw_mem = rows.row(row);
        if (want_texel_row) {
            const int* const l_tex_widths = late->sc.textures_widths;
            const int* const l_tex_starts = late->sc.textures_starts;
            tex_w = l_tex_widths[base + row]; tstart = l_tex_starts[base + row];
        }
    };
    auto finish_group = [&](const int q, const int r, const float rx, const float ry, const float rlen,
                            const float nearest_s, const int nearest_idx, const float4 hw_mem, const int tex_w, const int tstart) {
    const LateArgs late = late_args();
    const bool want_texel_row = COLOUR || (OBS && MS_WANTED(OUT_SEEN, late->out.seen_stamp));
    const bool want_line = want_texel_row || MS_WANTED(OUT_LOCATIONS, late->out.locations) || MS_WANTED(OUT_DOTS, late->out.dots);
    float loc = NAN, dt = NAN;
    float4 hw = make_float4(0.f, 0.f, 0.f, 0.f);
    if (want_line) {
        float4 aw = make_float4(0.f, 0.f, 0.f, 0.f);
        if (__ballot((nearest_idx >= 0) & (nearest_idx < AF))) aw = agent_line(nearest_idx);
        if (nearest_idx >= 0) {
            hw = (nearest_idx < AF) ? aw : hw_mem;
            const float vx = hw.z - hw.x, vy = hw.w - hw.y;
            const float d = rx*vy - ry*vx;
            const float pqx = hw.x - pp.x, pqy = hw.y - pp.y;
            loc = div_inrange(pqx*ry - pqy*rx, d);
            const float dtop = rx*vx + ry*vy;
            const float dbot = rlen*sqrt_any(vx*vx + vy*vy);
            dt = div_inrange(dtop, dbot + 1.e-6f);
        }
    }
    [[maybe_unused]] const size_t o = ((size_t)n*A + a)*R + r;
    const float dist = nearest_s*rlen;
    if constexpr (PLANES) {
        if (!MASKED || (out_mask_ & (OUT_INDICES | OUT_LOCATIONS | OUT_DOTS | OUT_DISTANCES))) {
            int* const o_indices = late->out.indices;
            float* const o_locations = late->out.locations;
            float* const o_dots = late->out.dots;
            float* const o_distances = late->out.distances;
            if (r < R) {
                if (!OBS || MS_WANTED(OUT_INDICES, o_indices)) __builtin_nontemporal_store(nearest_idx, &o_indices[o]);
                if (!OBS || MS_WANTED(OUT_LOCATIONS, o_locations)) __builtin_nontemporal_store(loc, &o_locations[o]);
                if (!OBS || MS_WANTED(OUT_DOTS, o_dots)) __builtin_nontemporal_store(dt, &o_dots[o]);
                if (!OBS || MS_WANTED(OUT_DISTANCES, o_distances)) __builtin_nontemporal_store(dist, &o_distances[o]);
            }
        }
    }

    const bool is_hit = (nearest_idx >= 0) & (r < R);
    float s0 = 0.f, s1 = 0.f, s2 = 0.f;
    [[maybe_unused]] Filt f = Filt{0, 0, 0.f, 0.f};
    [[maybe_unused]] float intensity = 0.f;
    [[maybe_unused]] float tl0 = 0.f, tl1 = 0.f, tl2 = 0.f, tr0 = 0.f, tr1 = 0.f, tr2 = 0.f;
    if constexpr (COLOUR) {
        const float* const l_tex_vals = late->sc.textures_vals;
        const float* const l_baked = late->sc.baked_vals;
        const bool dynamic = is_hit & (nearest_idx < AF);
        [[maybe_unused]] unsigned light_telemetry = 0x80000000u;
        if (__ballot(dynamic)) {
            if (sc.lg_vals) {
                __builtin_amdgcn_fence(__ATOMIC_RELEASE, "wavefront");
                __builtin_amdgcn_wave_barrier();
                const float cx_l = hw.x*(1 - loc) + hw.z*loc, cy_l = hw.y*(1 - loc) + hw.w*loc;
                const LightScene scl{sc.n_agents, sc.n_model, late->sc.lights_vals, late->sc.lights_widths, late->sc.lights_starts,
                                     late->sc.lg_vals, late->sc.lg_starts, late->sc.lg_geom, late->sc.lg_cell,
                                     late->sc.lg_list, late->sc.lg_pool, reinterpret_cast<const float4*>(late->sc.lg_pool_rows),
                                     rc.by_m.mul, rc.by_m.sh1, rc.by_m.sh2};
#if MS_PROBE
                unsigned lclk[2] = {0u, 0u};
                PROBE_VAL(14, (unsigned)clock64())
                intensity = grid_light_intensity(scl, ag, n, lane, dynamic, nearest_idx, cx_l, cy_l, L, ln,
                    reinterpret_cast<LightPair*>(&s_raw[O_EPI]), reinterpret_cast<unsigned*>(&s_raw[O_EPI + 2048]), light_telemetry, lclk);
                PROBE_VAL(12, lclk[0]) PROBE_VAL(13, lclk[1]) PROBE_VAL(11, (unsigned)clock64())
#else
                intensity = grid_light_intensity(scl, ag, n, lane, dynamic, nearest_idx, cx_l, cy_l, L, ln,
                    reinterpret_cast<LightPair*>(&s_raw[O_EPI]), reinterpret_cast<unsigned*>(&s_raw[O_EPI + 2048]), light_telemetry);
#endif
                PROBE_VAL(2, light_telemetry)
            } else if constexpr (NG == 1) {
                if (out.workspace && lane == 0) out.workspace[16 + atomicAdd(&out.workspace[0], 1)] = fan;
            }
        }
        PROBE_AT(5, tex_w)
        f = tex_filter(is_hit ? loc : 0.f, tex_w);
        const float bk_l = l_baked[tstart + f.l], bk_r = l_baked[tstart + f.r];
        const float* __restrict__ tl = l_tex_vals + 3*(size_t)(tstart + f.l);
        const float* __restrict__ tr = l_tex_vals + 3*(size_t)(tstart + f.r);
        tl0 = tl[0]; tl1 = tl[1]; tl2 = tl[2]; tr0 = tr[0]; tr1 = tr[1]; tr2 = tr[2];
        if (is_hit & !dynamic) intensity = f.lw*bk_l + f.rw*bk_r;
    }
    if constexpr (OBS >= 1) {
        if (MS_WANTED(OUT_SEEN, late->out.seen_stamp)) {
            bool fresh = false, fresh_last = false;
            const int last_env = sc.n_envs - 1;
            if (is_hit) {
                const float wf = (float)tex_w;
                const int along = (int)ms_min(floorf(wf*loc), wf - 1);
                const int epoch = late->out.seen_epoch[n];
                if (late->out.seen_stamp[tstart + along] != epoch)
                    fresh = atomicExch(&late->out.seen_stamp[tstart + along], epoch) != epoch;
            } else if ((r < R) & (sc.n_texels_total > 0)) {
                const int last = sc.n_texels_total - 1;
                const int epoch = late->out.seen_epoch[last_env];
                if (late->out.seen_stamp[last] != epoch)
                    fresh_last = atomicExch(&late->out.seen_stamp[last], epoch) != epoch;
            }
            const unsigned long long fm = __ballot(fresh);
            if (fm && lane == 0) atomicAdd(&late->out.seen_count[n], __popcll(fm));
            if (__ballot(fresh_last) && lane == 0) atomicAdd(&late->out.seen_count[last_env], 1);
        }
        if (MS_WANTED(OUT_CENTRE, late->out.obs_centre)) {
            const int sub = MASKED ? (late->out.obs_subsample & 0xff) : late->out.obs_subsample, sh = __builtin_ctz((unsigned)sub), W = R >> sh;
            const int r1 = (((W >> 1) - 1) << sh) + (sub >> 1), r2 = ((W >> 1) << sh) + (sub >> 1);
            if ((r == r1) | (r == r2)) {
                int seen = -1;
                if ((nearest_idx >= 0) & (nearest_idx < AF)) seen = div_by(nearest_idx, rc.by_m);
                late->out.obs_centre[((size_t)n*A + a)*2 + (r == r2 ? 1 : 0)] = seen;
            }
        }
    }

    if constexpr (COLOUR) {
        PROBE_AT(6, tl0)
        if (is_hit) {
            const float dn = 1 - dt*dt;
            s0 = dn*intensity*(f.lw*tl0 + f.rw*tr0);
            s1 = dn*intensity*(f.lw*tl1 + f.rw*tr1);
            s2 = dn*intensity*(f.lw*tl2 + f.rw*tr2);
        }
        if constexpr (PLANES) {
        float* const o_screen = late->out.screen;
        if (!OBS || MS_WANTED(OUT_SCREEN, o_screen)) {
            s_screen_w[3*lane] = s0; s_screen_w[3*lane + 1] = s1; s_screen_w[3*lane + 2] = s2;
            __builtin_amdgcn_fence(__ATOMIC_RELEASE, "wavefront");
            __builtin_amdgcn_wave_barrier();
            __builtin_amdgcn_fence(__ATOMIC_ACQUIRE, "wavefront");
            const int nfl = 3*min(n_live - q*WAVE, WAVE);
            float* __restrict__ scr = o_screen + 3*(((size_t)n*A + a)*R + r0 + q*WAVE);
            #pragma unroll
            for (int k = 0; k < 3; k++) {
                const int j = lane + k*WAVE;
                if (j < nfl) __builtin_nontemporal_store(s_screen_w[j], &scr[j]);
            }
        }
        }
    }
    if (OBS && ((COLOUR && MS_WANTED(OUT_RGB, late->out.obs_rgb)) || MS_WANTED(OUT_DEPTH, late->out.obs_depth))) {
        const int sub = MASKED ? (late->out.obs_subsample & 0xff) : late->out.obs_subsample;
        float p0 = s0, p1 = s1, p2 = s2;
        float pd = 1.f - ms_min(ms_max((dist - agent_radius)*late->out.obs_max_depth, 0.f), 1.f);
        auto quad_xor = [](const float v, auto ctrl) {
            return __int_as_float(__builtin_amdgcn_mov_dpp(__float_as_int(v), decltype(ctrl)::value, 0xf, 0xf, true));
        };
        constexpr std::integral_constant<int, 0xB1> XOR1{};
        constexpr std::integral_constant<int, 0x4E> XOR2{};
        if (sub > 1) {
            if constexpr (COLOUR) { p0 += quad_xor(p0, XOR1); p1 += quad_xor(p1, XOR1); p2 += quad_xor(p2, XOR1); }
            pd += quad_xor(pd, XOR1);
        }
        if (sub > 2) {
            if constexpr (COLOUR) { p0 += quad_xor(p0, XOR2); p1 += quad_xor(p1, XOR2); p2 += quad_xor(p2, XOR2); }
            pd += quad_xor(pd, XOR2);
        }
        for (int o2 = 4; o2 < sub; o2 <<= 1) {
            if constexpr (COLOUR) {
                p0 += __shfl_xor(p0, o2, WAVE); p1 += __shfl_xor(p1, o2, WAVE); p2 += __shfl_xor(p2, o2, WAVE);
            }
            pd += __shfl_xor(pd, o2, WAVE);
        }
        if (((lane & (sub - 1)) == 0) & (r < R)) {
            const int sh = __builtin_ctz((unsigned)sub);
            const float inv = bits_f((uint32_t)(127 - sh) << 23);
// ... 149 lines not shown
        int raw_pos = 0, q_len = 0, al_left = AL;
        int q_first = 0;
        for (;;) {
            while ((raw_pos < n_raw) & (q_len <= Q_CAP - WAVE)) {
                const unsigned e = e_next[0];
                e_next[0] = e_next[1];
                e_next[1] = raw(raw_pos + 2*WAVE);
                const int k = raw_pos + lane;
                const int idx = listed ? (int)(e & 0xffffu) : k;
                const bool keep = (k < n_raw) & (!listed | wg_arcs_meet((int)((e >> 16) & 255u), (int)(e >> 24), wa8, wb8));
                const unsigned long long km = __ballot(keep);
                if (keep) s_queue_w[q_len + (int)__builtin_amdgcn_mbcnt_hi((unsigned)(km >> 32), __builtin_amdgcn_mbcnt_lo((unsigned)km, 0u))] = (unsigned short)idx;
                q_len += __popcll(km);
                raw_pos += WAVE;
            }
            __builtin_amdgcn_fence(__ATOMIC_RELEASE, "wavefront");
            __builtin_amdgcn_wave_barrier();
            __builtin_amdgcn_fence(__ATOMIC_ACQUIRE, "wavefront");
            const int al0 = AL - al_left;
            const int n_al = min(al_left, AHEAD*WAVE);
            const int n_items = n_al + min(q_len, AHEAD*WAVE - n_al);
            const int q_used = n_items - n_al;
            int l_it[AHEAD];
            float4 w_it[AHEAD];
            #pragma unroll
            for (int kk = 0; kk < AHEAD; kk++) {
                const int i = kk*WAVE + lane;
                const int ai = al0 + i;
                const int q_at = min(max(i - n_al, 0), Q_CAP - 1);
                const int qe = listed ? (int)s_queue_w[q_at] : q_first + q_at;
                l_it[kk] = (i < n_al) ? ai + (ai >= own0 ? own : 0) : AF + qe;
                w_it[kk] = rows.load(l_it[kk]*16, 0);
            }
            PROBE_VAL(2, 0)
            PROBE_AT(3, w_it[0].x)
            #pragma unroll
            for (int kk = 0; kk < AHEAD; kk++) {
                if (kk*WAVE >= n_items) continue;
                admit_fn(w_it[kk], l_it[kk], kk*WAVE + lane < n_items, kk*WAVE < n_al, al0 + kk*WAVE == 0);
            }
            al_left -= n_al;
            __builtin_amdgcn_wave_barrier();
            if (q_used < q_len) {
                unsigned short keep_[Q_CAP/WAVE];
                #pragma unroll
                for (int j = 0; j < Q_CAP/WAVE; j++) keep_[j] = s_queue_w[min(q_used + j*WAVE + lane, Q_CAP - 1)];
                __builtin_amdgcn_wave_barrier();
                #pragma unroll
                for (int j = 0; j < Q_CAP/WAVE; j++) if (j*WAVE + lane < q_len - q_used) s_queue_w[j*WAVE + lane] = keep_[j];
            }
            q_len -= q_used;
            q_first += q_used;
            if (((raw_pos >= n_raw) & (q_len == 0) & (al_left == 0)) || stop_fn()) break;
        }
    };
    if constexpr (NG == 1) {
        walk(pa_last, pa_first, admit, [] { return false; });
        if (n_pairs) drain();
    }
    __builtin_amdgcn_fence(__ATOMIC_ACQUIRE, "wavefront");
    bool list_whole = true;
    auto resolve_group = [&](const int q, const float rx, const float ry, const float near, float& nearest_s, int& nearest_idx) {
        const unsigned long long best = s_best_w[lane], second = s_second_w[lane], third = s_third_w[lane];
        bool ambiguous = false;
        if (best != ~0ull) {
            const float s1 = bits_f((uint32_t)(best >> 32)), s2 = bits_f((uint32_t)(second >> 32)), s3 = bits_f((uint32_t)(third >> 32));
            const int i1 = (int)(uint32_t)best, i2 = (int)(uint32_t)second;
            nearest_s = s1;
            nearest_idx = i1;
            if ((second != ~0ull) && !(s1 < s2 - 1.e-4f)) {
                if ((third == ~0ull) || (s2 < s3 - 1.e-4f)) {
                    const bool first_is_1 = i1 < i2;
                    const float sa = first_is_1 ? s1 : s2, sb = first_is_1 ? s2 : s1;
                    const int ia = first_is_1 ? i1 : i2, ib = first_is_1 ? i2 : i1;
                    const bool b_wins = sb < sa - 1.e-4f;
                    nearest_s = b_wins ? sb : sa;
                    nearest_idx = b_wins ? ib : ia;
                } else {
                    ambiguous = true;
                }
            }
        }
        const unsigned long long amb = __ballot(ambiguous);
        PROBE_VAL(11, n_pairs_total) PROBE_VAL(12, n_drains == 1 ? list_n : -1) PROBE_VAL(13, __popcll(amb))
#if MS_PROBE
        const unsigned t_fold0 = (unsigned)clock64();
        PROBE_VAL(15, t_fold0)
#endif
        if (out.workspace && lane == 0 && q == 0 && rc.telemetry) {
            atomicAdd(&out.workspace[3], n_pairs_total); atomicAdd(&out.workspace[4], n_windows);
        }
        if (amb && out.workspace && lane == 0) {
            atomicAdd(&out.workspace[1], __popcll(amb));
            if (__popcll(amb) > 6) atomicAdd(&out.workspace[2], 1);
        }
        if (amb && (NG == 1 ? n_drains == 1 : list_whole)) {
            const int rounds = (list_n + WAVE - 1)/WAVE;
            if (2*(int)__popcll(amb)*rounds <= list_n + 16) {
                float x = INFINITY;
                int xi = -1;
                for (int k0 = 0; k0 < list_n; k0 += WAVE) {
                    const int k = min(k0 + lane, list_n - 1);
                    const Cand cd = s_cand_w[k];
                    const int line = s_info_w[k].y;
                    const float cpv = cd.pqx*cd.vy - cd.pqy*cd.vx;
                    for (unsigned long long todo = amb; todo; todo &= todo - 1) {
                        const int jr = __ffsll((long long)todo) - 1;
                        const float jrx = readlane_f(rx, jr), jry = readlane_f(ry, jr), jnear = readlane_f(near, jr);
                        const float d = jrx*cd.vy - jry*cd.vx;
                        const float nt = cd.pqx*jry - cd.pqy*jrx;
                        const float ad = fabsf(d);
                        const float ntp = bits_f(f_bits(nt) ^ (f_bits(d) & 0x80000000u));
                        bool valid = false;
                        float sv = 0.f;
                        if ((k0 + lane < list_n) & (ad >= 1.e-3f) & (ntp >= 0.f) & (ntp <= ad)) {
                            sv = div_inrange(cpv, d);
                            valid = jnear < sv;
                        }
                        unsigned long long m = __ballot(valid);
                        if (m) {
                            float xs = readlane_f(x, jr);
                            int xis = __builtin_amdgcn_readlane(xi, jr);
                            for (; m; m &= m - 1) {
                                const int j = __ffsll((long long)m) - 1;
                                const float sj = readlane_f(sv, j);
                                if (sj < xs - 1.e-4f) { xs = sj; xis = __builtin_amdgcn_readlane(line, j); }
                            }
                            if (lane == jr) { x = xs; xi = xis; }
                        }
                    }
                }
                if (ambiguous) { nearest_s = x; nearest_idx = xi; }
            } else {
                float x = INFINITY;
                int xi = -1;
                #pragma unroll 4
                for (int k = 0; k < list_n; k++) {
                    const Cand cd = s_cand_w[k];
                    const int line = s_info_w[k].y;
                    if (ambiguous) {
                        const float d = rx*cd.vy - ry*cd.vx;
                        const float nt = cd.pqx*ry - cd.pqy*rx;
                        const float ad = fabsf(d);
                        const float ntp = bits_f(f_bits(nt) ^ (f_bits(d) & 0x80000000u));
                        if ((ad >= 1.e-3f) & (ntp >= 0.f) & (ntp <= ad)) {
                            const float sv = div_inrange(cd.pqx*cd.vy - cd.pqy*cd.vx, d);
                            if ((near < sv) & (sv < x - 1.e-4f)) { x = sv; xi = line; }
                        }
                    }
                }
                if (ambiguous) { nearest_s = x; nearest_idx = xi; }
            }
        } else
        if (__popcll(amb) > 6) {
            float x = INFINITY;
            int xi = -1;
            for (int c0 = 0; c0 < L; c0 += WAVE) {
                Cand mine;
                int lo = 0, len = 0;
                line_math(fetch(c0), c0 + lane, c0 + lane < L, c0 < AF, NG == 1 && c0 == 0, mine, lo, len);
                __builtin_amdgcn_wave_barrier();
                s_cand_w[lane] = mine;
                __builtin_amdgcn_fence(__ATOMIC_RELEASE, "wavefront");
                __builtin_amdgcn_wave_barrier();
                __builtin_amdgcn_fence(__ATOMIC_ACQUIRE, "wavefront");
                for (unsigned long long todo = __ballot(len > 0); todo; todo &= todo - 1) {
// ... 171 lines not shown
            winner_of(ni, hw_mem, tex_w, tstart);
            finish_group(q, r0 + q*WAVE + lane, gx, gy, ray_len(gx, gy), ns, ni, hw_mem, tex_w, tstart);
            __builtin_amdgcn_wave_barrier();
        };
        bool overflow = false;
        {
            const float pa = span_of(0, n_groups);
            n_list = 0; list_whole = true;
            auto admit_shared = [&](const float4 w, const int l, const bool live, const bool agent_lines, const bool) {
                if (overflow) return;
                Cand cd;
                int lo = 0, len = 0;
                line_math(w, l, live, agent_lines, false, cd, lo, len);
                const bool seen = len > 0;
                const unsigned long long vm = __ballot(seen);
                if (!vm) return;
                const int chunk_lines = __popcll(vm);
                if (n_list + chunk_lines > V_CAP) { overflow = true; return; }
                if (seen) {
                    const int k = n_list + (int)__builtin_amdgcn_mbcnt_hi((unsigned)(vm >> 32), __builtin_amdgcn_mbcnt_lo((unsigned)vm, 0u));
                    s_cand_w[k] = cd;
                    s_info_w[k] = make_int2(lo | (len << 16), l);
                }
                n_list += chunk_lines;
            };
            walk(readlane_f(pa, 1), readlane_f(pa, 0), admit_shared, [&] { return overflow; });
        }
        if (!overflow) {
            #pragma unroll 1
            for (int q = 0; q < n_groups; q++) {
                LANE_AFRESH;
                if (q) load_agents();
                float gx, gy, gl, gn;
                setup_group(q, gx, gy, gl, gn);
                group_rest(q, q, gx, gy);
            }
        } else {
            #pragma unroll 1
            for (int q = 0; q < n_groups; q++) {
                LANE_AFRESH;
                if (q) load_agents();
                const float pa = span_of(q, 1);
                float gx, gy, gl, gn;
                setup_group(q, gx, gy, gl, gn);
                n_list = 0; list_whole = true;
                auto admit_one = [&](const float4 w, const int l, const bool live, const bool agent_lines, const bool) {
                    Cand cd;
                    int lo = 0, len = 0;
                    line_math(w, l, live, agent_lines, false, cd, lo, len);
                    const bool seen = len > 0;
                    const unsigned long long vm = __ballot(seen);
                    if (!vm) return;
                    const int chunk_lines = __popcll(vm);
                    if (n_list + chunk_lines > V_CAP) {
                        pass2_group(0);
                        n_list = 0; list_whole = false;
                    }
                    if (seen) {
                        const int k = n_list + (int)__builtin_amdgcn_mbcnt_hi((unsigned)(vm >> 32), __builtin_amdgcn_mbcnt_lo((unsigned)vm, 0u));
                        s_cand_w[k] = cd;
                        s_info_w[k] = make_int2(lo | (len << 16), l);
                    }
                    n_list += chunk_lines;
                };
                walk(readlane_f(pa, 1), readlane_f(pa, 0), admit_one, [] { return false; });
                const float2 back = s_ray_w[lane];
                group_rest(q, 0, back.x, back.y);
            }
        }
    }

    PROBE_AT(4, nearest_idx)
    if constexpr (NG == 1) {
        float4 hw_mem; int tex_w, tstart;
        winner_of(nearest_idx, hw_mem, tex_w, tstart);
        finish_group(0, r, rx, ry, rlen, nearest_s, nearest_idx, hw_mem, tex_w, tstart);
    }
    PROBE_DONE(fan)
#undef MS_WANTED
}


__global__ __launch_bounds__(WG) void dynlight_kernel(
        const MsScenery sc, const MsAgents ag, const MsRender out, const int R) {
    __shared__ LightPair s_pair[WAVES][PAIRS];
    __shared__ unsigned s_shadow[2*WAVE];

    const int tid = threadIdx.x, wave = tid >> 6, lane = tid & 63;
    int fan = blockIdx.x;
    if (out.workspace) {
        if (fan >= out.workspace[0]) return;
        fan = out.workspace[16 + fan];
    }
    const int A = sc.n_agents, AF = sc.n_agents*sc.n_model;
    const int G = (R + WAVE - 1)/WAVE, F = A*G;
    const int n = fan / F, rem = fan - n*F, a = rem / G, g = rem - a*G;
    const int r = g*WAVE + lane;
    const size_t o = ((size_t)n*A + a)*R + r;
    const int L = sc.lines_widths[n];
    const int base = sc.lines_starts[n];
    const int num_i = sc.lights_widths[n];
    const int lbase = sc.lights_starts[n];
    int nearest_idx = -1;
    float loc = 0.f, dt = 0.f;
    if (r < R) { nearest_idx = out.indices[o]; loc = out.locations[o]; dt = out.dots[o]; }
    const bool dynamic = (nearest_idx >= 0) & (nearest_idx < AF);
    const unsigned long long dyn = __ballot(dynamic);
    if (!dyn) return;

    const float4* __restrict__ ln = reinterpret_cast<const float4*>(sc.lines_vals) + base;
    const float* __restrict__ lights = sc.lights_vals + 3*(size_t)lbase;
    float4 hw = make_float4(0.f, 0.f, 0.f, 0.f);
    Filt f = Filt{0, 0, 0.f, 0.f};
    float t0[3] = {0.f, 0.f, 0.f}, t1[3] = {0.f, 0.f, 0.f};
    if (dynamic) {
        hw = ln[nearest_idx];
        const int start = base + nearest_idx;
        f = tex_filter(loc, sc.textures_widths[start]);
        const int tstart = sc.textures_starts[start];
        const float* __restrict__ tl = sc.textures_vals + 3*(size_t)(tstart + f.l);
        const float* __restrict__ tr = sc.textures_vals + 3*(size_t)(tstart + f.r);
        #pragma unroll
        for (int k = 0; k < 3; k++) { t0[k] = tl[k]; t1[k] = tr[k]; }
    }
    const float cx_l = hw.x*(1 - loc) + hw.z*loc, cy_l = hw.y*(1 - loc) + hw.w*loc;
    const int my_target = dynamic ? nearest_idx / sc.n_model : -1;

    float acc = AMBIENT;
    bool saturated = false;
    for (int i0 = 0; i0 < num_i; i0 += WAVE) {
        const int ni = min(WAVE, num_i - i0);
        float Ix = 0.f, Iy = 0.f, Ii = 0.f;
        if (lane < ni) { Ix = lights[3*(i0 + lane)]; Iy = lights[3*(i0 + lane) + 1]; Ii = lights[3*(i0 + lane) + 2]; }
        const bool shortcut = (num_i <= WAVE) & (__ballot((lane < ni) & !(Ii >= 0.f)) == 0ull);
        __syncthreads();
        if (wave == 0) { s_shadow[2*lane] = 0u; s_shadow[2*lane + 1] = 0u; }
        unsigned long long todo = dyn;
        while (todo) {
            const int j = __ffsll((long long)todo) - 1;
            const int target = __builtin_amdgcn_readlane(my_target, j);
            const bool mine = dynamic & (my_target == target);
            todo &= ~__ballot(mine);
            const float2 T = reinterpret_cast<const float2*>(ag.positions)[n*A + target];
            float rho = mine ? sqrtf((cx_l - T.x)*(cx_l - T.x) + (cy_l - T.y)*(cy_l - T.y)) : 0.f;
            rho = wave_max_f(rho) + 2e-3f + 1e-4f*(fabsf(T.x) + fabsf(T.y));
            const float dx = T.x - Ix, dy = T.y - Iy;
            const float key = dx*dx + dy*dy;
            const float el = sqrtf(key);
            const float ex = dx/el, ey = dy/el;
            int rank = 0;
            for (int q = 0; q < ni; q++) {
                const float kq = readlane_f(key, q);
                rank += ((kq < key) | ((kq == key) & (q < lane))) ? 1 : 0;
            }
            if (lane >= ni) rank = -1;
            auto ranked = [&](int oi) { return __ffsll((long long)__ballot(rank == oi)) - 1; };

            auto sweep = [&](int o_lo, int o_hi, unsigned long long open) {
                int cnt = 0;
                auto flush = [&]() {
                    __builtin_amdgcn_fence(__ATOMIC_RELEASE, "wavefront");
                    __builtin_amdgcn_wave_barrier();
                    __builtin_amdgcn_fence(__ATOMIC_ACQUIRE, "wavefront");
                    for (int p0 = 0; p0 < cnt; p0 += WAVE) {
                        const LightPair pr = s_pair[wave][min(p0 + lane, cnt - 1)];
                        const P2 I = p2(pr.ix, pr.iy);
                        for (unsigned long long rays = open; rays; rays &= rays - 1) {
// ... 81 lines not shown
```

megastep_amd/csrc/megastep_hip.hip:

```cpp
#include <hip/hip_runtime.h>
#include <math.h>
#include <stdint.h>
#include <stddef.h>
#include <stdlib.h>
#include <string.h>
#include <atomic>
#include "../../include/megastep_hip_test.h"

namespace {

constexpr float AMBIENT = .1f;
constexpr float LUMINANCE = 2.f;
constexpr int WAVE = 64;
constexpr int WG = 256;
constexpr int WAVES = WG/WAVE;

thread_local int g_last_hip_error = 0;
thread_local int g_pair_telemetry = 0;
thread_local int g_ray_groups = 0;
thread_local int g_physics_pack = 0;
thread_local float g_tail_rounds = -1.f;
thread_local int g_tail_envs = -1;
thread_local int g_last_step_fused = 0;
thread_local int g_last_render_groups = 0;
thread_local int g_overhead_cull = 1;

#ifndef MS_PROBE
#define MS_PROBE 0
#endif
#if MS_PROBE
constexpr int PROBE_STAMPS = 8;
constexpr int PROBE_WORDS = 16;
__device__ unsigned* g_probe = nullptr;
__device__ long long g_probe_cap = 0;
struct Probe {
    unsigned t = 0u, real0 = (unsigned)wall_clock64();
    __device__ void done(const int lane, const long long wave) {
        if (g_probe && wave < g_probe_cap) {
            unsigned v = t;
            if (lane == PROBE_STAMPS) v = ((unsigned)__builtin_amdgcn_s_getreg((31 << 11) | 4) & 0xffffu) | ((unsigned)(__builtin_amdgcn_s_getreg((3 << 11) | 20) & 0xf) << 16);
            if (lane == PROBE_STAMPS + 1) v = real0;
            if (lane == PROBE_STAMPS + 2) v = (unsigned)wall_clock64();
            if (lane < PROBE_WORDS) g_probe[wave*PROBE_WORDS + lane] = v;
        }
    }
};
#define PROBE_STAMP(k) { const unsigned c_ = (unsigned)clock64(); asm volatile("v_writelane_b32 %0, %1, " #k : "+v"(probe_.t) : "s"(c_)); }
#define PROBE_INIT Probe probe_; PROBE_STAMP(0)
#define PROBE_AT(i, v) { asm volatile("" :: "v"(v)); PROBE_STAMP(i) }
#define PROBE_DONE(wave) { PROBE_STAMP(7) probe_.done(lane, (long long)(wave)); }
#define PROBE_VAL(k, x) { const unsigned c_ = (unsigned)__builtin_amdgcn_readfirstlane((int)(x)); asm volatile("v_writelane_b32 %0, %1, " #k : "+v"(probe_.t) : "s"(c_)); }
#else
#define PROBE_INIT
#define PROBE_AT(i, v)
#define PROBE_DONE(tag)
#define PROBE_VAL(k, x)
#endif

#include "kernels/math.h"
#include "kernels/physics.h"
#include "kernels/lighting.h"
#include "kernels/render.h"
#include "kernels/bake.h"
#include "kernels/wallgrid.h"
#include "kernels/raycast.h"
#include "kernels/overhead.h"
#include "kernels/navfield.h"
#include "kernels/envlogic.h"

struct RenderPlan { int ng; long long n_blocks; };
RenderPlan render_plan(const int n_envs, const int n_agents, const int R, const int slots, const int pinned, const float tail_rounds,
                       const int tail_envs_exact, RenderConsts& rc) {
    int ng = 1;
    if (R >= 4*WAVE && 2LL*n_envs*n_agents*((R + 4*WAVE - 1)/(4*WAVE)) >= 5LL*slots) ng = 4;
    if (pinned == 1 || pinned == 2 || pinned == 4) ng = pinned;
    int tail = 0;
    const int G1 = (R + WAVE - 1)/WAVE;
    const int envs_lo = n_envs/8, envs_rem = n_envs % 8, envs_hi = envs_lo + (envs_rem ? 1 : 0);
    if (ng > 1) {
        const double rounds = tail_rounds >= 0.f ? (double)tail_rounds : 0.5;
        const long long tail_envs = tail_envs_exact >= 0 ? tail_envs_exact : (long long)ceil(rounds*slots*ng/((double)n_agents*G1));
        tail = (int)std::min<long long>((tail_envs + 7)/8, envs_hi);
        if (tail >= envs_hi && !(pinned > 1)) ng = 1;
    }
    const int G = (R + ng*WAVE - 1)/(ng*WAVE);
    rc.by_f = divisor_of((unsigned)(n_agents*G));
    rc.by_g = divisor_of((unsigned)G);
    rc.by_f1 = divisor_of((unsigned)(n_agents*G1));
    rc.by_g1 = divisor_of((unsigned)G1);
    rc.envs_lo = envs_lo; rc.envs_rem = envs_rem; rc.tail = tail;
    const long long n_blocks = ng > 1 ? 8LL*((long long)(envs_hi - std::min(tail, envs_hi))*n_agents*G + (long long)std::min(tail, envs_hi)*n_agents*G1)
                                      : (long long)n_envs*n_agents*G;
    return RenderPlan{ng, n_blocks};
}

int physics_pack_of(const int n_envs, const int n_agents, const bool gridded, const int pinned) {
    int pack = 1;
    if (gridded && n_agents <= 16) {
        pack = n_envs > 6144 ? std::min((n_envs + 4095)/4096, 16) : n_envs >= 3072 ? 2 : 1;
        pack = std::max(std::min(pack, WAVE/2/n_agents), 1);
    }
    if (pinned >= 1) pack = (gridded && (long long)pinned*n_agents <= WAVE) ? pinned : 1;
    return pack;
}

int hip_fail(hipError_t e) { g_last_hip_error = (int)e; return MS_EHIP; }
int launch_status() { const hipError_t e = hipGetLastError(); return e == hipSuccess ? MS_OK : hip_fail(e); }

int wave_slots_here() {
    constexpr int MAX_DEVICES = 64;
    static std::atomic<int> slots_of[MAX_DEVICES];
    int dev = 0;
    if (hipGetDevice(&dev) != hipSuccess) return 256*4*MS_WAVES;
    if (dev >= 0 && dev < MAX_DEVICES) { const int known = slots_of[dev].load(std::memory_order_relaxed); if (known) return known; }
    int cus = 0;
    if (hipDeviceGetAttribute(&cus, hipDeviceAttributeMultiprocessorCount, dev) != hipSuccess || cus <= 0) cus = 256;
    const int slots = cus*4*MS_WAVES_WIDE;
    if (dev >= 0 && dev < MAX_DEVICES) slots_of[dev].store(slots, std::memory_order_relaxed);
    return slots;
}

bool scenery_ok(const MsScenery* s) {
    return s && s->n_envs > 0 && s->n_agents > 0 && s->n_model > 0 && s->lines_vals && s->lines_widths &&
           s->lines_starts && s->model && ((uintptr_t)s->lines_vals % 16 == 0) && ((uintptr_t)s->model % 16 == 0);
}
bool agents_ok(const MsAgents* a) { return a && a->angles && a->positions && a->angvelocity && a->velocity; }
bool config_ok(const MsConfig* c) {
    return c && c->res > 0 && c->fps > 0.f && c->agent_radius > 0.f && c->fov > 0.f && c->fov < 180.f;
}
MsAgents agents_or_none(const MsAgents* a) { return a ? *a : MsAgents{nullptr, nullptr, nullptr, nullptr, nullptr}; }

float half_screen_of(const float fov) { return tanf(3.14159265358979323846f/180.f*fov/2.); }

bool light_grid_in(const MsScenery* sc) { return sc->lg_vals && sc->lg_starts && sc->lg_geom && sc->lg_cell > 0.f; }
bool vis_lists_serve(const MsScenery* sc, const float near_plane) {
    return sc->wg_cells && sc->wg_starts && sc->wg_geom && sc->wg_pool && sc->wg_pool_base && sc->wg_cell > 0.f &&
           near_plane*1.001f < sc->wg_near;
}

bool step_options_ok(const MsMovement* mv, const MsStepExtras* ex) {
    if (mv && (!mv->actions || !mv->table || mv->n_actions < 1 || !(mv->keep == mv->keep))) return false;
    if (ex) {
        if (ex->spawn_positions && (!ex->spawn_angles || !ex->respawn_mask || !ex->respawn_choice || ex->n_spawns < 1 ||
                                    ((uintptr_t)ex->spawn_positions % 8))) return false;
        if (ex->lifespans && (!ex->max_lifespans || !ex->fresh_max)) return false;
        if (ex->imu && !(ex->imu_ang_scale == ex->imu_ang_scale && ex->imu_speed_scale == ex->imu_speed_scale)) return false;
    }
    return true;
}
void step_options_of(const MsMovement* mv, const MsStepExtras* ex, MsMovement& mvv, MsStepExtras& exv) {
    mvv = mv ? *mv : MsMovement{nullptr, nullptr, 0, 0.f};
    exv = ex ? *ex : MsStepExtras{nullptr, nullptr, nullptr, nullptr, 0, 0, nullptr, nullptr, nullptr, nullptr, 1.f, 1.f};
    exv.imu_ang_scale = 1.f/exv.imu_ang_scale; exv.imu_speed_scale = 1.f/exv.imu_speed_scale;
}

}

extern "C" {

int ms_abi_version(void) { return MS_ABI_VERSION; }

const char* ms_strerror(int code) {
    switch (code) {
        case MS_OK: return "ok";
        case MS_EINVAL: return "invalid argument (null/misaligned pointer, non-positive size or bad config)";
        case MS_EHIP: return "a HIP runtime call failed (see ms_last_hip_error)";
        case MS_EUNSUPPORTED: return "shape not supported by the gfx950 kernels";
        case MS_ENODEVICE: return "no HIP device visible";
        default: return "unknown megastep_hip error";
    }
}

int ms_last_hip_error(void) { return g_last_hip_error; }

int ms_device_count(void) {
    int n = 0;
    const hipError_t e = hipGetDeviceCount(&n);
    if (e != hipSuccess || n <= 0) { g_last_hip_error = (int)e; return MS_ENODEVICE; }
    return n;
}

void ms_host_sincospi(float x, float* s, float* c) { sincospi_f(x, *s, *c); }

int ms_host_bake_point_bin(float light_x, float light_y, float x, float y) { return bake_point_bin(p2(light_x, light_y), p2(x, y)); }
void ms_host_bake_wall_bins(float light_x, float light_y, float ax, float ay, float bx, float by, int* first, int* count) {
    bake_wall_bins(p2(light_x, light_y), ax, ay, bx, by, *first, *count);
}

#if MS_PROBE
int ms_debug_probe(unsigned* buf, long long capacity) {
    if (hipMemcpyToSymbol(HIP_SYMBOL(g_probe), &buf, sizeof buf) != hipSuccess) return hip_fail(hipGetLastError());
    if (hipMemcpyToSymbol(HIP_SYMBOL(g_probe_cap), &capacity, sizeof capacity) != hipSuccess) return hip_fail(hipGetLastError());
    return MS_OK;
}
#endif

int ms_debug_ray_groups(int groups) { g_ray_groups = groups; return MS_OK; }
int ms_debug_last_render_groups(void) { return g_last_render_groups; }
int ms_debug_physics_pack(int envs) { g_physics_pack = envs; return MS_OK; }
int ms_host_physics_pack(int n_envs, int n_agents, int gridded, int pinned) { return physics_pack_of(n_envs, n_agents, gridded != 0, pinned); }
long long ms_host_render_plan(int n_envs, int n_agents, int res, int slots, int pinned_groups, float tail_rounds, int tail_envs, int* groups) {
    RenderConsts rc;
    const RenderPlan plan = render_plan(n_envs, n_agents, res, slots, pinned_groups, tail_rounds, tail_envs, rc);
    if (groups) *groups = plan.ng;
    return plan.n_blocks;
}
int ms_host_render_block(int n_envs, int n_agents, int res, int slots, int pinned_groups, float tail_rounds, int tail_envs, long long block, int* out4) {
    RenderConsts rc;
    const RenderPlan plan = render_plan(n_envs, n_agents, res, slots, pinned_groups, tail_rounds, tail_envs, rc);
    int fan = 0;
    if (block < 0 || block >= plan.n_blocks) return -1;
    return render_block((int)block, (int)plan.n_blocks, n_agents, res, plan.ng, rc, out4[0], out4[1], out4[2], out4[3], fan) ? 1 : 0;
}
int ms_debug_ray_group_tail(float rounds, int envs) { g_tail_rounds = rounds; g_tail_envs = envs; return MS_OK; }
int ms_debug_pair_telemetry(int on) { g_pair_telemetry = on ? 1 : 0; return MS_OK; }

int ms_test_arithmetic(const float* n, const float* d, float* q_inrange, float* q_ieee, const float* x, float* r_any, float* r_ieee,
                       long long count, void* stream) {
    if (count < 0 || ((q_inrange || q_ieee) && !(n && d)) || ((r_any || r_ieee) && !x)) return MS_EINVAL;
    if (count == 0) return MS_OK;
    const long long blocks = (count + WG - 1)/WG;
    if (blocks > 0x7fffffffLL) return MS_EUNSUPPORTED;
    hipLaunchKernelGGL(arithmetic_test_kernel, dim3((unsigned)blocks), dim3(WG), 0, (hipStream_t)stream, n, d, q_inrange, q_ieee, x, r_any, r_ieee, count);
    return launch_status();
}

void ms_host_ray_interval_wide(const float* pose, const float* line, int res, float fov, float agent_radius, int groups, int wave,
                               int* first, int* count) {
    const float half_screen = half_screen_of(fov);
    const float x_clip = 0.5f*agent_radius/sqrtf(1.f + half_screen*half_screen), c_b = 0.5f*(float)res/half_screen;
    const int nr = WAVE*groups, r0 = wave*nr;
    const float c_a = 0.5f*((float)res - 1.f), g0 = (float)r0;
    const int r_last = (r0 + nr - 1 < res - 1) ? r0 + nr - 1 : res - 1;
    const float last_local = (float)(r_last - r0);
    float xa, ya, xb, yb;
    agent_frame(pose[3], pose[2], line[0] - pose[0], line[1] - pose[1], line[2] - pose[0], line[3] - pose[1], xa, ya, xb, yb);
    ray_interval(xa, ya, xb, yb, true, x_clip, c_a, c_b, g0, last_local, *first, *count, (float)nr);
}
void ms_host_ray_interval(const float* pose, const float* line, int res, float fov, float agent_radius, int group, int* first, int* count) {
    ms_host_ray_interval_wide(pose, line, res, fov, agent_radius, 1, group, first, count);
}

int ms_host_lightgrid_cell(const float* walls, int n_walls, const float* lights, int n_lights, float ox, float oy, int nx, int ny,
                           float cell, int c, unsigned* words, unsigned* candidates, int max_candidates) {
    const LgCell k = lg_cell_of(make_float4(ox, oy, (float)nx, (float)ny), cell, c);
    const int num_i = n_lights < LG_LIGHTS ? n_lights : LG_LIGHTS;
    words[0] = words[1] = words[2] = words[3] = 0u;
    int count = 0;
    for (int i = 0; i < num_i; i++) {
        const LgView v = lg_view_of(k, p2(lights[3*i], lights[3*i + 1]));
        bool touched = false, dark = false;
        for (int j = 0; j < n_walls && !dark; j++) {
            const float4 w = make_float4(walls[4*j], walls[4*j + 1], walls[4*j + 2] - walls[4*j], walls[4*j + 3] - walls[4*j + 1]);
            if (!lg_touches(k, v, w)) continue;
            touched = true;
            dark = lg_shadows(v, w);
        }
        const unsigned st = dark ? 2u : (touched ? 0u : 1u);
        words[i >> 4] |= st << (2*(i & 15));
        if (st == 0u) {
            for (int j = 0; j < n_walls; j++) {
                const float4 w = make_float4(walls[4*j], walls[4*j + 1], walls[4*j + 2] - walls[4*j], walls[4*j + 3] - walls[4*j + 1]);
                if (!lg_touches(k, v, w)) continue;
                if (count < max_candidates) candidates[count] = 0x80000000u | ((unsigned)i << 24) | (unsigned)j;
                count++;
            }
        }
    }
    return count;
}

int ms_host_fold_hits(const float* s, const int* line, int n_hits, const int* order, float* nearest_s, int* nearest_line) {
    unsigned long long best = ~0ull, second = ~0ull, third = ~0ull;
    for (int w0 = 0; w0 < n_hits; w0 += WAVE) {
        const int nw = (n_hits - w0 < WAVE) ? n_hits - w0 : WAVE;
        unsigned long long lose1[WAVE], lose2[WAVE];
        bool on[WAVE];
        for (int k = 0; k < nw; k++) {
            const int h = order[w0 + k];
            const unsigned long long key = hit_key(s[h], line[h]);
            on[k] = hit_loser_matters(key, s[h], slot_min(&best, key), lose1[k]);
        }
        for (int k = 0; k < nw; k++) if (on[k]) {
            const unsigned long long old2 = slot_min(&second, lose1[k]);
            lose2[k] = old2 > lose1[k] ? old2 : lose1[k];
        }
        for (int k = 0; k < nw; k++) if (on[k] && lose2[k] != ~0ull) slot_min(&third, lose2[k]);
    }
    *nearest_s = INFINITY; *nearest_line = -1;
    return hit_resolve(best, second, third, *nearest_s, *nearest_line) ? 1 : 0;
}

float ms_host_wall_reach(const float* agent, float agent_radius) { return wall_reach(p2(agent[0], agent[1]), p2(agent[2], agent[3]), agent_radius); }

int ms_host_wall_beyond_reach(const float* agent, const float* wall, float agent_radius) {
    const float reach = wall_reach(p2(agent[0], agent[1]), p2(agent[2], agent[3]), agent_radius);
    return wall_beyond(make_float4(agent[0], agent[1], agent[2], agent[3]), make_float4(wall[0], wall[1], wall[2], wall[3]),
                       reach_squared(reach)) ? 1 : 0;
}

int ms_host_agents_apart(const float* me, const float* other, float agent_radius) {
    return agents_apart(make_float4(me[0], me[1], me[2], me[3]), make_float4(other[0], other[1], other[2], other[3]), agent_radius) ? 1 : 0;
}

int ms_host_wall_hidden(float x0, float y0, float x1, float y1, const float* o, const float* w, float near_plane) {
    const WgCell k{x0, y0, x1, y1};
    const WgTarget t = wg_target(k, make_float4(w[0], w[1], w[2], w[3]));
    return wg_hides(k, t, make_float4(o[0], o[1], o[2], o[3]), near_plane) ? 1 : 0;
}

void ms_host_wallgrid_cell(const float* walls, int n_walls, float ox, float oy, int nx, int ny, float cell, int c,
                           float near_plane, float reach_lo, float reach, unsigned char* vis, unsigned char* close) {
    const float4* ln = reinterpret_cast<const float4*>(walls);
    const WgCell k = wg_cell_of(make_float4(ox, oy, (float)nx, (float)ny), cell, c);
    for (int t = 0; t < n_walls; t++) {
        const WgTarget tg = wg_target(k, ln[t]);
        bool hidden = false;
        for (int o = 0; o < n_walls && !hidden; o++) hidden = (o != t) && wg_hides(k, tg, ln[o], near_plane);
        vis[t] = hidden ? 0 : 1;
        close[t] = wg_close(k, ln[t], reach) ? (wg_close(k, ln[t], reach_lo) ? 2 : 1) : 0;
    }
}

void ms_host_wall_sectors(float x0, float y0, float x1, float y1, const float* o, int* first, int* count, const float* w, int* sector) {
    const float cx = .5f*(x0 + x1), cy = .5f*(y0 + y1);
    wg_sectors_of(cx, cy, make_float4(o[0], o[1], o[2], o[3]), *first, *count);
    *sector = wg_sector_of(cx, cy, make_float4(w[0], w[1], w[2], w[3]));
}
void ms_host_wall_arc(float x0, float y0, float x1, float y1, const float* w, int* lo8, int* hi8) {
    wg_arc(WgCell{x0, y0, x1, y1}, make_float4(w[0], w[1], w[2], w[3]), *lo8, *hi8);
}
int ms_host_wedge_meets(float right_x, float right_y, float left_x, float left_y, int lo8, int hi8) {
    int wa8, wb8;
    wg_wedge(pseudo_angle(right_x, right_y), pseudo_angle(left_x, left_y), wa8, wb8);
    return wg_arcs_meet(lo8, hi8, wa8, wb8) ? 1 : 0;
}

static bool wallgrid_ok(const MsScenery* sc) {
    return sc->wg_starts && sc->wg_geom && sc->wg_cell > 0.f && sc->wg_reach_lo >= 0.f && sc->wg_reach >= sc->wg_reach_lo &&
           sc->wg_near > 0.f && ((uintptr_t)sc->wg_geom % 16 == 0);
}

int ms_wallgrid_scan(const MsScenery* sc, const MsWallGridParent* parent, const int* reps, int n_reps, int max_groups,
                     const long long* bits_starts, unsigned* bits, unsigned* counts, void* stream) {
    if (!scenery_ok(sc) || !wallgrid_ok(sc) || !reps || n_reps < 0 || max_groups < 0 || !bits_starts || !bits || !counts) return MS_EINVAL;
    WgParent par{nullptr, nullptr, nullptr, 0.f, nullptr};
    if (parent) {
        if (!parent->cells || !parent->starts || !parent->geom || !parent->pool || !(parent->cell >= sc->wg_cell) ||
            ((uintptr_t)parent->cells % 16) || ((uintptr_t)parent->geom % 16)) return MS_EINVAL;
        par = WgParent{parent->cells, parent->starts, parent->geom, parent->cell, parent->pool};
    }
    if (n_reps == 0 || max_groups == 0) return MS_OK;
    if (n_reps > 65535) return MS_EUNSUPPORTED;
    hipLaunchKernelGGL(wallgrid_scan_kernel, dim3((unsigned)max_groups, (unsigned)n_reps), dim3(WG), 0, (hipStream_t)stream,
                       *sc, par, reps, bits_starts, bits, counts);
    return launch_status();
}

int ms_wallgrid_fill(const MsScenery* sc, const int* reps, int n_reps, int max_cells,
                     const long long* bits_starts, const unsigned* bits, unsigned short* pool, unsigned* vis_entries, float* near_rows,
                     void* stream) {
    if (!scenery_ok(sc) || !wallgrid_ok(sc) || !sc->wg_cells || ((uintptr_t)sc->wg_cells % 16) || !reps || n_reps < 0 || max_cells < 0 ||
        !bits_starts || !bits || ((vis_entries != nullptr) != (near_rows != nullptr)) || (!pool && !vis_entries) || (vis_entries && !sc->wg_pool_base) ||
        ((uintptr_t)near_rows % 16) || ((uintptr_t)vis_entries % 4)) return MS_EINVAL;
    if (n_reps == 0 || max_cells == 0) return MS_OK;
    const long long blocks = (2LL*max_cells + WAVES - 1)/WAVES;
    if (blocks > 0x7fffffffLL || n_reps > 65535) return MS_EUNSUPPORTED;
    hipLaunchKernelGGL(wallgrid_fill_kernel, dim3((unsigned)blocks, (unsigned)n_reps), dim3(WG), 0, (hipStream_t)stream,
                       *sc, reps, bits_starts, bits, pool, reinterpret_cast<float4*>(near_rows), vis_entries);
    return launch_status();
}

int ms_step_physics(const MsScenery* sc, const MsAgents* ag, const MsMovement* mv, const MsStepExtras* ex, float* progress,
                    const MsConfig* cfg, void* stream) {
    if (!scenery_ok(sc) || !agents_ok(ag) || !progress || !config_ok(cfg)) return MS_EINVAL;
    if (!step_options_ok(mv, ex)) return MS_EINVAL;
    if (sc->wg_cells && (!sc->wg_starts || !sc->wg_geom || !sc->wg_near_rows || !(sc->wg_cell > 0.f) || ((uintptr_t)sc->wg_cells % 16) ||
                         ((uintptr_t)sc->wg_geom % 16) || ((uintptr_t)sc->wg_near_rows % 16))) return MS_EINVAL;
    const int pack = physics_pack_of(sc->n_envs, sc->n_agents, sc->wg_cells != nullptr, g_physics_pack);
    const size_t slice = ((sizeof(float)*8 + sizeof(float) + sizeof(unsigned))*(size_t)sc->n_agents*pack + 15)/16;
    if (slice*16 > 56*1024) return MS_EUNSUPPORTED;
    MsMovement mvv; MsStepExtras exv;
    step_options_of(mv, ex, mvv, exv);
    MsScenery scn = *sc;
    if (!sc->wg_cells) { scn.wg_geom = sc->lines_vals; scn.wg_starts = sc->lines_starts; }
    const hipStream_t hs = (hipStream_t)stream;
    const Divisor by_a = divisor_of((unsigned)sc->n_agents);
#define MS_LAUNCH_PHYSICS_P(M, E, P) \
    hipLaunchKernelGGL((physics_kernel<M, E, P>), dim3((sc->n_envs + pack - 1)/pack), dim3(WAVE), slice*16, hs, scn, *ag, progress, cfg->agent_radius, cfg->fps, mvv, exv, pack, by_a)
#define MS_LAUNCH_PHYSICS(M, E) { if (pack > 1) MS_LAUNCH_PHYSICS_P(M, E, 1); else MS_LAUNCH_PHYSICS_P(M, E, 0); }
    if (mv && ex) MS_LAUNCH_PHYSICS(1, 1)
    else if (ex) MS_LAUNCH_PHYSICS(0, 1)
    else if (mv) MS_LAUNCH_PHYSICS(1, 0)
    else MS_LAUNCH_PHYSICS(0, 0)
#undef MS_LAUNCH_PHYSICS_P
#undef MS_LAUNCH_PHYSICS
    return launch_status();
}

int ms_move_physics(const MsScenery* sc, const MsAgents* ag, const MsMovement* mv, float* progress, const MsConfig* cfg,
                    void* stream) {
    return ms_step_physics(sc, ag, mv, nullptr, progress, cfg, stream);
}

int ms_physics(const MsScenery* sc, const MsAgents* ag, float* progress, const MsConfig* cfg, void* stream) {
    return ms_step_physics(sc, ag, nullptr, nullptr, progress, cfg, stream);
}

struct RenderLaunch {
    RenderPlan plan;
    RenderConstsStep rc;
    MsScenery scn; MsAgents agn; MsRender outn;
    const MsAgents* ag; const MsRender* out;
    float agent_radius, half_screen; int R;
    bool colour, obs, no_planes;
    bool light_grid, walls_listed;
    bool prep;
    bool dynlight;
    bool fused;
};

static int render_prepare(const MsScenery* sc, const MsAgents* ag, const MsRender* out, const MsConfig* cfg, float* progress,
                          const MsMovement* mv, const MsStepExtras* ex, RenderLaunch& L) {
    if (!scenery_ok(sc) || !agents_ok(ag) || !config_ok(cfg) || !out || !sc->textures_vals || !sc->textures_widths ||
        !sc->textures_starts || !sc->baked_vals || !sc->lights_widths || !sc->lights_starts) return MS_EINVAL;
    if ((out->seen_stamp != nullptr) != (out->seen_epoch != nullptr) || (out->seen_stamp != nullptr) != (out->seen_count != nullptr)) return MS_EINVAL;
    if (out->obs_rgb || out->obs_depth || out->obs_centre) {
        const int sub = out->obs_subsample;
        if (sub < 1 || (sub & (sub - 1)) || sub > WAVE || cfg->res % sub) return MS_EINVAL;
        if (out->obs_depth && !(out->obs_max_depth > 0.f)) return MS_EINVAL;
        if (out->obs_centre && cfg->res/sub < 2) return MS_EINVAL;
    }
    if (sc->n_lights_total > 0 && !sc->lights_vals) return MS_EINVAL;
    const int R = cfg->res;
    L.R = R; L.agent_radius = cfg->agent_radius; L.ag = ag; L.out = out;
    L.light_grid = light_grid_in(sc);
    L.colour = out->screen || out->obs_rgb;
    L.dynlight = !L.light_grid && sc->n_agents > 1 && L.colour;
    L.plan = render_plan(sc->n_envs, sc->n_agents, R, wave_slots_here(), L.dynlight ? 1 : g_ray_groups, g_tail_rounds, g_tail_envs, L.rc);
    const long long ws_queue = (long long)sc->n_envs*sc->n_agents*((R + WAVE - 1)/WAVE);
    if (L.plan.n_blocks > 0x7fffffffLL || ws_queue > 0x7fffff00LL) return MS_EUNSUPPORTED;
    L.rc.ws_headings = 16 + (int)((ws_queue + 1) & ~1LL);
    const float half_screen = L.half_screen = half_screen_of(cfg->fov);
    L.scn = *sc;
    if (!L.light_grid) L.scn.lg_vals = nullptr;
    L.walls_listed = vis_lists_serve(sc, cfg->agent_radius) && 1.f + half_screen*half_screen <= WG_MAX_RU2;
    if (L.walls_listed && (((uintptr_t)sc->wg_cells % 16) || ((uintptr_t)sc->wg_geom % 16))) return MS_EINVAL;
    if (!L.walls_listed) {
        L.scn.wg_cells = nullptr;
        L.scn.wg_geom = sc->lines_vals;
        L.scn.wg_starts = sc->lines_starts;
        L.scn.wg_pool_base = reinterpret_cast<const long long*>(sc->lines_vals);
    }
    const bool all_planes = out->indices && out->locations && out->dots && out->distances && out->screen;
    const bool pooled = out->obs_rgb || out->obs_depth || out->obs_centre || out->seen_stamp;
    if (L.dynlight && (!all_planes || pooled)) return MS_EUNSUPPORTED;
    if (!pooled && !out->indices && !out->locations && !out->dots && !out->distances && !out->screen) return MS_EINVAL;
    L.obs = pooled || !all_planes;
    L.no_planes = L.colour && !out->indices && !out->locations && !out->dots && !out->distances && !out->screen;
    const bool physics_listed = sc->wg_cells != nullptr;
    L.fused = progress && sc->n_agents == 1 && R <= WAVE && L.plan.ng == 1 && physics_listed == L.walls_listed &&
              (!physics_listed || (sc->wg_near_rows && (uintptr_t)sc->wg_near_rows % 16 == 0));
    const bool cached = ag->headings && !L.dynlight;
    L.prep = !cached && !L.fused && out->workspace;
    if ((cached && (uintptr_t)ag->headings % 16) || (L.prep && (uintptr_t)out->workspace % 8)) return MS_EINVAL;
    L.agn = *ag;
    L.outn = *out;
    if (!cached && !L.fused) L.agn.headings = nullptr;
    if (!L.prep) L.outn.workspace = nullptr;
    if (out->obs_depth) L.outn.obs_max_depth = 1.f/out->obs_max_depth;
    L.rc.x_clip = 0.5f*cfg->agent_radius/sqrtf(1.f + half_screen*half_screen);
    L.rc.c_b = 0.5f*(float)R/half_screen;
    L.rc.by_m = divisor_of((unsigned)sc->n_model);
    L.rc.skip_own = (sc->model_radius > 0.f && sc->model_radius*1.01f < cfg->agent_radius) ? 1 : 0;
    L.rc.inv_res = camera_inv_res(R, half_screen);
    L.rc.telemetry = g_pair_telemetry;
    if (!L.colour || (L.obs && L.plan.ng == 1))
        L.outn.obs_subsample = (out->obs_subsample & 0xff) | (((out->indices ? OUT_INDICES : 0) | (out->locations ? OUT_LOCATIONS : 0) |
                                (out->dots ? OUT_DOTS : 0) | (out->distances ? OUT_DISTANCES : 0) | (out->obs_depth ? OUT_DEPTH : 0) |
                                (out->obs_centre ? OUT_CENTRE : 0) | (out->seen_stamp ? OUT_SEEN : 0) | (out->screen ? OUT_SCREEN : 0) |
                                (out->obs_rgb ? OUT_RGB : 0)) << 8);
    if (L.fused) {
        L.rc.progress = progress; L.rc.fps = cfg->fps; L.rc.wg_cells_physics = sc->wg_cells;
        step_options_of(mv, ex, L.rc.mv, L.rc.ex);
    }
    return MS_OK;
}

static int render_enqueue(const RenderLaunch& L, const hipStream_t hs) {
    g_last_render_groups = L.plan.ng;
    const int na = L.scn.n_envs*L.scn.n_agents;
    if (L.prep) hipLaunchKernelGGL(render_prep_kernel, dim3((na + WG - 1)/WG), dim3(WG), 0, hs, *L.ag, L.out->workspace, na, L.rc.ws_headings);
#define MS_LAUNCH_RENDER(O, S, NG_, STEP_) hipLaunchKernelGGL((render_kernel<O, S, NG_, STEP_>), dim3((int)L.plan.n_blocks), dim3(WAVE), 0, hs, \
                                                              L.scn, L.agn, L.outn, L.agent_radius, L.half_screen, L.R, (int)L.plan.n_blocks, L.rc)
#define MS_LAUNCH_RENDER_OS(NG_) { if (!L.colour) MS_LAUNCH_RENDER(1, 0, NG_, 0); else if (L.no_planes) MS_LAUNCH_RENDER(2, 1, NG_, 0); \
                                   else if (L.obs) MS_LAUNCH_RENDER(1, 1, NG_, 0); else MS_LAUNCH_RENDER(0, 1, NG_, 0); }
    if (L.fused) { if (!L.colour) MS_LAUNCH_RENDER(1, 0, 1, 1); else if (L.obs) MS_LAUNCH_RENDER(1, 1, 1, 1); else MS_LAUNCH_RENDER(0, 1, 1, 1); }
    else if (L.plan.ng == 4) MS_LAUNCH_RENDER_OS(4)
    else if (L.plan.ng == 2) MS_LAUNCH_RENDER_OS(2)
    else MS_LAUNCH_RENDER_OS(1)
#undef MS_LAUNCH_RENDER_OS
#undef MS_LAUNCH_RENDER
    if (L.dynlight) hipLaunchKernelGGL(dynlight_kernel, dim3((int)L.plan.n_blocks), dim3(WG), 0, hs, L.scn, *L.ag, *L.out, L.R);
    return launch_status();
}

int ms_deathmatch_shoot(int n_envs, int n_agents, const MsDeathmatch* dm, void* stream) {
    if (n_envs <= 0 || n_agents <= 0 || !dm || !dm->centre || !dm->positions || !dm->upper || !dm->health || !dm->damage || !dm->dead ||
        ((uintptr_t)dm->centre % 8) || ((uintptr_t)dm->positions % 8) || ((uintptr_t)dm->upper % 8) ||
        !(dm->clearance == dm->clearance) || !(dm->hit_damage == dm->hit_damage) || !(dm->tick_damage == dm->tick_damage)) return MS_EINVAL;
    const long long rows = (long long)n_envs*n_agents, blocks = (rows + WG - 1)/WG;
    if (blocks > 0x7fffffffLL) return MS_EUNSUPPORTED;
    hipLaunchKernelGGL(deathmatch_kernel, dim3((unsigned)blocks), dim3(WG), 0, (hipStream_t)stream, *dm, n_envs, n_agents);
    return launch_status();
}

int ms_explorer_books(int n_envs, const MsExplorer* ex, void* stream) {
    if (n_envs <= 0 || !ex || !ex->tally || !ex->before || !ex->lengths || !ex->epoch || !ex->over || !ex->reward || ex->pixels <= 0 ||
        ((uintptr_t)ex->tally % 4) || ((uintptr_t)ex->before % 4) || ((uintptr_t)ex->lengths % 4) || ((uintptr_t)ex->epoch % 4)) return MS_EINVAL;
    hipLaunchKernelGGL(explorer_kernel, dim3((unsigned)((n_envs + WG - 1)/WG)), dim3(WG), 0, (hipStream_t)stream, *ex, n_envs);
    return launch_status();
}

int ms_render(const MsScenery* sc, const MsAgents* ag, const MsRender* out, const MsConfig* cfg, void* stream) {
    RenderLaunch L;
    const int planned = render_prepare(sc, ag, out, cfg, nullptr, nullptr, nullptr, L);
    return planned != MS_OK ? planned : render_enqueue(L, (hipStream_t)stream);
}

int ms_move_step_render(const MsScenery* sc, const MsAgents* ag, const MsMovement* mv, const MsStepExtras* ex, float* progress,
                        const MsRender* out, const MsConfig* cfg, void* stream) {
    if (!progress || !step_options_ok(mv, ex)) return MS_EINVAL;
    RenderLaunch L;
    const int planned = render_prepare(sc, ag, out, cfg, progress, mv, ex, L);
    g_last_step_fused = 0;
    if (planned != MS_OK) return planned;
    const int p = L.fused ? MS_OK : ms_step_physics(sc, ag, mv, ex, progress, cfg, stream);
    const int r = p != MS_OK ? p : render_enqueue(L, (hipStream_t)stream);
    g_last_step_fused = L.fused && r == MS_OK;
    return r;
}
int ms_step_render(const MsScenery* sc, const MsAgents* ag, float* progress, const MsRender* out, const MsConfig* cfg, void* stream) {
    return ms_move_step_render(sc, ag, nullptr, nullptr, progress, out, cfg, stream);
}
int ms_debug_last_step_fused(void) { return g_last_step_fused; }

int ms_raycast(const MsScenery* sc, const MsAgents* ag, const MsRaycast* rq, const MsConfig* cfg, void* stream) {
    (void)cfg;
    if (!scenery_ok(sc) || !rq || rq->n_rays < 1 || !rq->origins || !rq->dirs || !(rq->near_plane >= 0.f) ||
        ((uintptr_t)rq->origins % 8) || ((uintptr_t)rq->dirs % 8)) return MS_EINVAL;
    if (ag && (!ag->angles || !ag->positions || ((uintptr_t)ag->positions % 8))) return MS_EINVAL;
    const long long total = (long long)sc->n_envs*rq->n_rays;
    if (total > 0x7fffff00LL) return MS_EUNSUPPORTED;
    const bool gridded = vis_lists_serve(sc, rq->near_plane);
    if (gridded && (((uintptr_t)sc->wg_cells % 16) || ((uintptr_t)sc->wg_geom % 16))) return MS_EINVAL;
    const unsigned blocks = (unsigned)((total + WG - 1)/WG);
    hipLaunchKernelGGL(raycast_kernel, dim3(blocks), dim3(WG), 0, (hipStream_t)stream, *sc, agents_or_none(ag), *rq, ag ? 1 : 0,
                       gridded ? 1 : 0, (int)total);
    return launch_status();
}

int ms_camera_rays(const MsAgents* ag, int n_envs, int n_agents, const MsConfig* cfg, float* dirs, void* stream) {
    if (!ag || !ag->angles || n_envs < 1 || n_agents < 1 || !config_ok(cfg) || !dirs || ((uintptr_t)dirs % 8)) return MS_EINVAL;
    const long long total = (long long)n_envs*n_agents*cfg->res;
    if ((long long)n_envs*n_agents > 0x7fffffffLL || total > 0x7fffff00LL*(long long)WG) return MS_EUNSUPPORTED;
    const float half_screen = half_screen_of(cfg->fov);
    hipLaunchKernelGGL(camera_rays_kernel, dim3((unsigned)((total + WG - 1)/WG)), dim3(WG), 0, (hipStream_t)stream, ag->angles,
                       n_envs*n_agents, cfg->res, half_screen, camera_inv_res(cfg->res, half_screen), reinterpret_cast<float2*>(dirs));
    return launch_status();
}

int ms_overhead(const MsScenery* sc, const MsAgents* ag, const MsOverhead* ov, void* stream) {
    if (!scenery_ok(sc) || !ov || ov->n_images < 1 || ov->n_views < 1 || ov->height < 1 || ov->width < 1 || !ov->views ||
        (!ov->rgb && !ov->indices) || !(ov->half_width >= 0.f) || !(ov->half_width < INFINITY)) return MS_EINVAL;
    if (ov->rgb && (!sc->textures_vals || !sc->textures_widths || !sc->textures_starts || (ov->lit && !sc->baked_vals))) return MS_EINVAL;
    if (ag && (!ag->angles || !ag->positions || ((uintptr_t)ag->positions % 8))) return MS_EINVAL;
    if (ov->height > (1 << 15) || ov->width > (1 << 15)) return MS_EUNSUPPORTED;
    OvArgs a;
    a.envs = ov->envs; a.views = ov->views; a.rgb = ov->rgb; a.indices = ov->indices;
    a.n_views = ov->n_views; a.height = ov->height; a.width = ov->width;
    a.tiles_x = (ov->width + OV_TILE - 1)/OV_TILE; a.tiles_y = (ov->height + OV_TILE - 1)/OV_TILE;
    a.half_width = ov->half_width; a.h2 = ov->half_width*ov->half_width;
    a.bg_r = ov->background[0]; a.bg_g = ov->background[1]; a.bg_b = ov->background[2];
    a.lit = ov->lit ? 1 : 0; a.with_agents = ag ? 1 : 0; a.cull = g_overhead_cull ? 1 : 0;
    const long long total = (long long)ov->n_images*ov->n_views*a.tiles_x*a.tiles_y;
    const long long per_launch = 1LL << 22;
// ... 93 lines not shown
```

megastep_amd/cuda.py:

```python
import ctypes as C
import math
import numbers
import os
import torch
from . import _lib, grids
from ._lib import _on, _stream

_config = None


_switched = __import__('threading').local()


def _ab_switches():
    if getattr(_switched, 'done', False):
        return
    _switched.done = True
    g = os.environ.get('MEGASTEP_RAY_GROUPS')
    if g:
        _lib.lib().ms_debug_ray_groups(int(g))
    k = os.environ.get('MEGASTEP_PHYSICS_PACK')
    if k:
        _lib.lib().ms_debug_physics_pack(int(k))
    t, e = os.environ.get('MEGASTEP_RAY_GROUP_TAIL'), os.environ.get('MEGASTEP_RAY_GROUP_TAIL_ENVS')
    if t or e:
        _lib.lib().ms_debug_ray_group_tail(float(t) if t else -1., int(e) if e else -1)


def config(agent_radius, res, fov, fps):
    if not (0 < fov < 180):
        raise RuntimeError('fov must be in (0, 180) degrees')
    if res <= 0 or fps <= 0 or agent_radius <= 0:
        raise RuntimeError('agent_radius, res and fps must be positive')
    return _lib.MsConfig(float(agent_radius), int(res), float(fov), float(fps))


def initialize(agent_radius, res, fov, fps):
    global _config
    _config = config(agent_radius, res, fov, fps)
    _ab_switches()


def _cfg(agents=None, explicit=None):
    if explicit is not None:
        if not isinstance(explicit, _lib.MsConfig):
            raise RuntimeError('config must come from megastep_amd.cuda.config(agent_radius, res, fov, fps)')
        return explicit
    own = getattr(agents, '_config', None)
    if own is not None:
        return own
    if _config is None:
        raise RuntimeError('megastep_amd.cuda.initialize(agent_radius, res, fov, fps) has not been called')
    return _config


def _check(t, name, dtype, ndim):
    if not isinstance(t, torch.Tensor):
        raise RuntimeError(f'{name} must be a tensor')
    if not t.is_contiguous():
        raise RuntimeError(f'{name} must be contiguous')
    if t.dtype != dtype:
        raise RuntimeError(f'{name} must have dtype {dtype}, not {t.dtype}')
    if t.ndim != ndim:
        raise RuntimeError(f'{name} must be {ndim}-dimensional, not {t.ndim}')
    return t


def _require_gpu(*tensors):
    dev = tensors[0].device
    for t in tensors:
        if not t.is_cuda:
            raise RuntimeError('megastep_amd kernels need GPU (HIP) tensors; got a tensor on ' + str(t.device))
        if t.device != dev:
            raise RuntimeError(f'all tensors must live on one device; got {t.device} and {dev}')
    return dev


class _Ragged:
    _ndim = None

    def __init__(self, vals, widths):
        _check(vals, 'vals', torch.float32, self._ndim)
        _check(widths, 'widths', torch.int32, 1)
        if vals.device != widths.device:
            raise RuntimeError('vals and widths must be on the same device')
        ends = widths.cumsum(0).to(torch.int32)
        total = int(ends[-1]) if len(widths) else 0
        if total != vals.shape[0]:
            raise RuntimeError(f'widths sum to {total} but vals has {vals.shape[0]} rows')
        self._vals, self._widths = vals, widths
        self._starts, self._ends = ends - widths, ends
        self._inverse = torch.repeat_interleave(
            torch.arange(len(widths), dtype=torch.int32, device=widths.device), widths.long())

    vals = property(lambda self: self._vals)
    widths = property(lambda self: self._widths)
    starts = property(lambda self: self._starts)
    ends = property(lambda self: self._ends)
    inverse = property(lambda self: self._inverse)

    def __len__(self):
        return len(self._widths)

    def __getitem__(self, x):
        if isinstance(x, numbers.Integral):
            return self._vals[int(self._starts[x]):int(self._ends[x])]
        if isinstance(x, slice):
            start, stop, step = x.indices(len(self._widths))
            if step != 1:
                raise IndexError('Ragged slices must have step 1')
            if stop <= start:
                return type(self)(self._vals[:0], self._widths[:0])
            return type(self)(self._vals[int(self._starts[start]):int(self._ends[stop - 1])], self._widths[start:stop])
        raise TypeError(f"Can't index a Ragged with a {type(x).__name__}")

    def size(self, i):
        return self._vals.shape[i]

    def clone(self):
        return type(self)(self._vals.clone(), self._widths.clone())

    def numpyify(self):
        from .ragged import RaggedNumpy
        return RaggedNumpy(self._vals.detach().cpu().numpy().copy(), self._widths.detach().cpu().numpy().copy())

    def to(self, device):
        return type(self)(self._vals.to(device), self._widths.to(device))

    def __repr__(self):
        return f'{type(self).__name__}(vals={tuple(self._vals.shape)}, widths=({len(self._widths)},))'


class Ragged1D(_Ragged):
    _ndim = 1


class Ragged2D(_Ragged):
    _ndim = 2


class Ragged3D(_Ragged):
    _ndim = 3


class Agents:

    HEADING_CACHE = True

    def __init__(self, angles, positions, angvelocity, velocity, config=None):
        self._config = config
        self._angles = _check(angles, 'angles', torch.float32, 2)
        self._positions = _check(positions, 'positions', torch.float32, 3)
        self._angvelocity = _check(angvelocity, 'angvelocity', torch.float32, 2)
        self._velocity = _check(velocity, 'velocity', torch.float32, 3)
        n, a = angles.shape
        if positions.shape != (n, a, 2) or velocity.shape != (n, a, 2) or angvelocity.shape != (n, a):
            raise RuntimeError('agent tensors must be (N, A), (N, A, 2), (N, A), (N, A, 2)')
        self._headings = torch.full((n, a, 4), float('nan'), dtype=torch.float32, device=angles.device)
        ptrs = (angles.data_ptr(), positions.data_ptr(), angvelocity.data_ptr(), velocity.data_ptr())
        self._struct = _lib.MsAgents(*ptrs, self._headings.data_ptr())
        self._plain = _lib.MsAgents(*ptrs, None)
        self._cached = False
        self._epoch = 0
        self._use_cache = bool(self.HEADING_CACHE)
        devices = {t.device for t in (angles, positions, angvelocity, velocity)}
        self._dev = devices.pop() if len(devices) == 1 else None

    angles = property(lambda self: self._angles)
    positions = property(lambda self: self._positions)
    angvelocity = property(lambda self: self._angvelocity)
    velocity = property(lambda self: self._velocity)

    def state(self, e):
        from . import arrdict
        return arrdict.arrdict(angles=self._angles[e], positions=self._positions[e],
                               angvelocity=self._angvelocity[e], velocity=self._velocity[e])


class Scenery:

    def __init__(self, n_agents, lights, lines, textures, model, geom=None):
        if not isinstance(lights, Ragged2D) or not isinstance(lines, Ragged3D) or not isinstance(textures, Ragged2D):
            raise RuntimeError('lights, lines, textures must be Ragged2D, Ragged3D, Ragged2D')
        _check(model, 'model', torch.float32, 3)
        if lights.vals.shape[1:] != (3,) or lines.vals.shape[1:] != (2, 2) or textures.vals.shape[1:] != (3,) \
                or model.shape[1:] != (2, 2):
            raise RuntimeError('lights/lines/textures/model rows must be (3,), (2, 2), (3,), (2, 2)')
        if len(lights) != len(lines):
            raise RuntimeError('lights and lines must have one row per env')
        if len(textures) != lines.vals.shape[0]:
            raise RuntimeError('textures must have one row per line')
        self._n_agents = int(n_agents)
        self._lights, self._lines, self._textures, self._model = lights, lines, textures, model
        self._baked = Ragged1D(torch.ones_like(textures.vals[:, 0]).contiguous(), textures.widths)
        radius = float(model.reshape(-1, 2).norm(dim=1).max()) if model.numel() else 0.
        self._model_radius = radius if radius == radius and radius < float('inf') else 0.
        if geom is not None:
            _check(geom, 'geom', torch.int32, 1)
            if len(geom) != len(lines) or geom.device != lines.vals.device:
                raise RuntimeError('geom must have one entry per env, on the same device as the lines')
        self._geom = geom
        self._struct = None
        self._lg = None
        self._lg_decided = False
        self._wg_sum = None
        self._wg_weights = None
        self._wg = None
        self._wg_report = self._lg_report = None
        self._dev = None

    n_agents = property(lambda self: self._n_agents)
    lights = property(lambda self: self._lights)
    lines = property(lambda self: self._lines)
    textures = property(lambda self: self._textures)
    model = property(lambda self: self._model)
    baked = property(lambda self: self._baked)
    geom = property(lambda self: self._geom)

    def state(self, e):
        from . import dotdict
        s, t = int(self._lines.starts[e]), int(self._lines.ends[e])
        return dotdict.dotdict(n_agents=self._n_agents, lights=self._lights[e], lines=self._lines[e],
                               textures=self._textures[s:t], model=self._model, baked=self._baked[s:t])

    LIGHT_GRID = True
    LIGHT_GRID_CELL = float(os.environ.get('MEGASTEP_LIGHT_GRID_CELL', .125))
    LIGHT_GRID_POOL = 12
    LIGHT_GRID_BYTES = int(float(os.environ['MEGASTEP_LIGHT_GRID_BYTES'])) if os.environ.get('MEGASTEP_LIGHT_GRID_BYTES') else None

    WALL_GRID = os.environ.get('MEGASTEP_WALL_GRID', '1') != '0'
    WALL_GRID_CELL = float(os.environ.get('MEGASTEP_WALL_GRID_CELL', .25))
    WALL_GRID_REACH = (.7, 1.3)
    WALL_GRID_NEAR = .12
    WALL_GRID_BYTES = int(float(os.environ['MEGASTEP_WALL_GRID_BYTES'])) if os.environ.get('MEGASTEP_WALL_GRID_BYTES') else None
    WALL_GRID_MAX_CELLS = 1 << 18
    WALL_GRID_SCRATCH = 1 << 30
    WALL_GRID_COARSE = 4

    def grid_report(self):
        marks = getattr(self, '_bake_marks', None)
        if getattr(self, '_bake_s', None) is None and marks is not None and marks[0] is not None:
            ev, wall_grid = marks
            ev[2].synchronize()
            self._bake_s = dict(lighting=ev[0].elapsed_time(ev[1])*1e-3, wall_grid=ev[1].elapsed_time(ev[2])*1e-3 if wall_grid else 0.)
# ... 712 lines not shown
```

Before: 98.96 million.

## Order render fans by last-frame cost using a counting sort in physics

The render kernel now records a per-fan cost estimate from the previous frame: lighting work, window count, list length and ambiguous rays. Extra wave-blocks prepended to the physics launch bucket-sort these costs into 64 classes, per XCD run, in descending order. The single-group render kernel then reads its fan from that schedule rather than a fixed slot mapping, so expensive fans start first and tail imbalance is reduced. The cost is extra physics blocks, an indirect load per render block, and a possible loss of spatial locality between neighbouring fans.

```diff
diff --git a/include/megastep_hip.h b/include/megastep_hip.h
--- a/include/megastep_hip.h
+++ b/include/megastep_hip.h
@@ -67,6 +67,7 @@
     float* angvelocity;
     float* velocity;
     float* headings;
+    int* schedule;
 } MsAgents;
 
 typedef struct MsRender {
diff --git a/megastep_amd/_lib.py b/megastep_amd/_lib.py
--- a/megastep_amd/_lib.py
+++ b/megastep_amd/_lib.py
@@ -40,7 +40,7 @@
 
 class MsAgents(C.Structure):
     _fields_ = [('angles', C.c_void_p), ('positions', C.c_void_p), ('angvelocity', C.c_void_p), ('velocity', C.c_void_p),
-                ('headings', C.c_void_p)]
+                ('headings', C.c_void_p), ('schedule', C.c_void_p)]
 
 
 class MsMovement(C.Structure):
@@ -99,7 +99,7 @@
                 ('out', C.c_void_p)]
 
 
-SYMBOLS = ('ms_host_ray_interval_wide', 'ms_debug_ray_groups', 'ms_debug_last_render_groups', 'ms_debug_last_step_fused', 'ms_step_render', 'ms_move_step_render', 'ms_debug_ray_group_tail', 'ms_debug_physics_pack', 'ms_host_render_plan', 'ms_host_render_block', 'ms_host_physics_pack', 'ms_debug_pair_telemetry', 'ms_test_arithmetic', 'ms_abi_version', 'ms_strerror', 'ms_last_hip_error', 'ms_device_count', 'ms_bake', 'ms_physics', 'ms_move_physics',
+SYMBOLS = ('ms_host_ray_interval_wide', 'ms_debug_render_order', 'ms_host_order_fans', 'ms_debug_ray_groups', 'ms_debug_last_render_groups', 'ms_debug_last_step_fused', 'ms_step_render', 'ms_move_step_render', 'ms_debug_ray_group_tail', 'ms_debug_physics_pack', 'ms_host_render_plan', 'ms_host_render_block', 'ms_host_physics_pack', 'ms_debug_pair_telemetry', 'ms_test_arithmetic', 'ms_abi_version', 'ms_strerror', 'ms_last_hip_error', 'ms_device_count', 'ms_bake', 'ms_physics', 'ms_move_physics',
            'ms_step_physics', 'ms_deathmatch_shoot', 'ms_explorer_books',
            'ms_render', 'ms_raycast', 'ms_camera_rays', 'ms_overhead', 'ms_nav_free', 'ms_nav_fields', 'ms_nav_query', 'ms_debug_overhead_cull', 'ms_host_overhead_keeps', 'ms_host_sincospi', 'ms_host_bake_point_bin', 'ms_host_bake_wall_bins',
            'ms_wallgrid_scan', 'ms_wallgrid_fill', 'ms_host_wall_hidden', 'ms_host_wall_sectors', 'ms_host_wallgrid_cell', 'ms_host_wall_arc',
@@ -228,6 +228,10 @@
         handle.ms_host_physics_pack.argtypes = [C.c_int, C.c_int, C.c_int, C.c_int]
         handle.ms_host_physics_pack.restype = C.c_int
         handle.ms_debug_ray_group_tail.restype = C.c_int
+        handle.ms_debug_render_order.argtypes = [C.c_int]
+        handle.ms_debug_render_order.restype = C.c_int
+        handle.ms_host_order_fans.argtypes = [C.c_int, _i32p, _i32p]
+        handle.ms_host_order_fans.restype = C.c_int
         handle.ms_debug_pair_telemetry.argtypes = [C.c_int]
         handle.ms_debug_pair_telemetry.restype = C.c_int
         handle.ms_test_arithmetic.argtypes = [C.c_void_p]*7 + [C.c_longlong, C.c_void_p]
diff --git a/megastep_amd/csrc/kernels/lighting.h b/megastep_amd/csrc/kernels/lighting.h
--- a/megastep_amd/csrc/kernels/lighting.h
+++ b/megastep_amd/csrc/kernels/lighting.h
@@ -24,7 +24,7 @@
 };
 
 __device__ inline float grid_light_intensity(
-        const LightScene sc, const MsAgents& ag, const int n, const int lane, const bool dynamic, const int nearest_idx,
+        const LightScene sc, const AgentsK& ag, const int n, const int lane, const bool dynamic, const int nearest_idx,
         const float cx_l, const float cy_l, const int L, const float4* __restrict__ ln,
         LightPair* s_pair, unsigned* s_shadow, unsigned& telemetry, [[maybe_unused]] unsigned* clk = nullptr) {
 #if MS_PROBE
diff --git a/megastep_amd/csrc/kernels/overhead.h b/megastep_amd/csrc/kernels/overhead.h
--- a/megastep_amd/csrc/kernels/overhead.h
+++ b/megastep_amd/csrc/kernels/overhead.h
@@ -63,7 +63,7 @@
     if ((d2 <= h2) & ((d2 < b.d2) | ((d2 == b.d2) & (l < b.idx)))) { b.d2 = d2; b.idx = l; b.t = t; }
 }
 
-__global__ __launch_bounds__(WG) void overhead_kernel(const MsScenery sc, const MsAgents ag, const OvArgs a) {
+__global__ __launch_bounds__(WG) void overhead_kernel(const MsScenery sc, const AgentsK ag, const OvArgs a) {
     __shared__ float4 s_rows[OV_CHUNK];
     __shared__ int s_idx[OV_CHUNK];
     __shared__ int s_wave[WAVES];
diff --git a/megastep_amd/csrc/kernels/physics.h b/megastep_amd/csrc/kernels/physics.h
--- a/megastep_amd/csrc/kernels/physics.h
+++ b/megastep_amd/csrc/kernels/physics.h
@@ -36,17 +36,79 @@
     return make_float3(w*ex.imu_ang_scale, (c_*v.x + s_*v.y)*ex.imu_speed_scale, (-s_*v.x + c_*v.y)*ex.imu_speed_scale);
 }
 
+constexpr int FAN_CLASSES = 64;
+constexpr int FAN_SORT_EACH = 8;
+constexpr int FAN_SORT_MAX = FAN_SORT_EACH*WAVE;
+struct FanSort { int* schedule; int n_fans, per_run, n_blocks; };
+__host__ __device__ inline int fan_class(const int cost) { return (unsigned)cost < (unsigned)(FAN_CLASSES - 1) ? cost : FAN_CLASSES - 1; }
+__host__ inline int fan_sort_per_run(const int n_fans) { return ((n_fans >> 3) + ((n_fans & 7) ? 1 : 0) + FAN_SORT_MAX - 1)/FAN_SORT_MAX; }
+__host__ __device__ inline void fan_sort_part(const int n_fans, const int K, const int block, int& first_fan, int& count, int& first_slot) {
+    const int xcd = block/K, k = block - xcd*K;
+    const int q8 = n_fans >> 3, r8 = n_fans & 7;
+    const int run = xcd*q8 + (xcd < r8 ? xcd : r8), len = q8 + (xcd < r8 ? 1 : 0);
+    const int lo = len/K, rem = len - lo*K;
+    count = lo + (k < rem ? 1 : 0);
+    first_fan = run + k*lo + (k < rem ? k : rem);
+    first_slot = run + k;
+}
+__device__ inline void fan_sort_wave(const FanSort fs, const int block, const int lane, int* s_cnt) {
+    int first_fan, count, first_slot;
+    fan_sort_part(fs.n_fans, fs.per_run, block, first_fan, count, first_slot);
+    const int* __restrict__ costs = fs.schedule;
+    int* __restrict__ order = fs.schedule + fs.n_fans;
+    s_cnt[lane] = 0;
+    int cls[FAN_SORT_EACH];
+    #pragma unroll
+    for (int j = 0; j < FAN_SORT_EACH; j++) {
+        const int i = j*WAVE + lane;
+        cls[j] = fan_class(costs[first_fan + (i < count ? i : 0)]);
+    }
+    __builtin_amdgcn_fence(__ATOMIC_RELEASE, "wavefront");
+    __builtin_amdgcn_wave_barrier();
+    #pragma unroll
+    for (int j = 0; j < FAN_SORT_EACH; j++) if (j*WAVE + lane < count) atomicAdd(&s_cnt[cls[j]], 1);
+    __builtin_amdgcn_fence(__ATOMIC_RELEASE, "wavefront");
+    __builtin_amdgcn_wave_barrier();
+    __builtin_amdgcn_fence(__ATOMIC_ACQUIRE, "wavefront");
+    const int mine = s_cnt[FAN_CLASSES - 1 - lane];
+    const int incl = wave_scan_add(mine);
+    __builtin_amdgcn_wave_barrier();
+    s_cnt[FAN_CLASSES - 1 - lane] = incl - mine;
+    __builtin_amdgcn_fence(__ATOMIC_RELEASE, "wavefront");
+    __builtin_amdgcn_wave_barrier();
+    __builtin_amdgcn_fence(__ATOMIC_ACQUIRE, "wavefront");
+    #pragma unroll
+    for (int j = 0; j < FAN_SORT_EACH; j++) {
+        const int i = j*WAVE + lane;
+        if (i < count) {
+            const int rank = atomicAdd(&s_cnt[cls[j]], 1);
+            order[first_slot + fs.per_run*rank] = first_fan + i;
+        }
+    }
+}
+
 template <int MOVE, int EXTRA, int PACK = 0>
 __global__ __launch_bounds__(WAVE) void physics_kernel(
-        const MsScenery sc, const MsAgents ag, float* __restrict__ progress,
-        const float agent_radius, const float fps, const MsMovement mv, const MsStepExtras ex, const int pack_envs, const Divisor by_a) {
-    PROBE_INIT
+        const MsScenery sc, const AgentsK ag, float* __restrict__ progress,
+        const float agent_radius, const float fps, const MsMovement mv, const MsStepExtras ex, const int pack_envs, const Divisor by_a,
+        const FanSort fs) {
     extern __shared__ float4 s_dyn[];
     __shared__ float4 s_wall[PHYS_PAIRS];
     __shared__ int s_tag[PHYS_PAIRS];
+    static_assert(PHYS_PAIRS >= FAN_CLASSES, "a sort wave's counts fit a physics wave's LDS");
+    int n_sort = fs.n_blocks;
+    asm("" : "+s"(n_sort) : "s"(sc.n_envs), "s"(sc.n_agents), "s"(sc.n_model), "s"(sc.wg_geom), "s"(sc.wg_starts), "s"(sc.wg_cells),
+                            "s"(sc.lines_vals), "s"(sc.lines_widths), "s"(sc.lines_starts), "s"(ag.positions), "s"(ag.velocity),
+                            "s"(pack_envs), "s"(by_a.mul), "s"(by_a.sh1), "s"(by_a.sh2));
+    if ((int)blockIdx.x < n_sort) {
+        fan_sort_wave(fs, blockIdx.x, threadIdx.x, s_tag);
+        return;
+    }
+    PROBE_INIT
     const int A1 = sc.n_agents, AF = sc.n_agents*sc.n_model;
     const int lane = threadIdx.x;
-    const int n = PACK ? blockIdx.x*pack_envs : blockIdx.x;
+    const int blk = blockIdx.x - n_sort;
+    const int n = PACK ? blk*pack_envs : blk;
     const int E = PACK ? min(pack_envs, sc.n_envs - n) : 1;
     const int A = PACK ? A1*E : A1;
     const int nA = n*A1;
diff --git a/megastep_amd/csrc/kernels/raycast.h b/megastep_amd/csrc/kernels/raycast.h
--- a/megastep_amd/csrc/kernels/raycast.h
+++ b/megastep_amd/csrc/kernels/raycast.h
@@ -15,7 +15,7 @@
     }
 }
 
-__global__ __launch_bounds__(WG) void raycast_kernel(const MsScenery sc, const MsAgents ag, const MsRaycast q, const int with_agents,
+__global__ __launch_bounds__(WG) void raycast_kernel(const MsScenery sc, const AgentsK ag, const MsRaycast q, const int with_agents,
                                                      const int gridded, const int n_total) {
     const int i_raw = blockIdx.x*WG + threadIdx.x;
     const bool live = i_raw < n_total;
diff --git a/megastep_amd/csrc/kernels/render.h b/megastep_amd/csrc/kernels/render.h
--- a/megastep_amd/csrc/kernels/render.h
+++ b/megastep_amd/csrc/kernels/render.h
@@ -32,7 +32,7 @@
     const float2 p = reinterpret_cast<const float2*>(positions)[n*n_agents + a];
     return drawn_row(s, c, p.x, p.y, reinterpret_cast<const float4*>(model)[m]);
 }
-__device__ inline float4 drawn_line(const MsScenery& sc, const MsAgents& ag, int n, int l) {
+__device__ inline float4 drawn_line(const MsScenery& sc, const AgentsK& ag, int n, int l) {
     return drawn_line_of(ag.angles, ag.positions, sc.model, sc.n_agents, sc.n_model, n, l);
 }
 
@@ -83,6 +83,9 @@
     MsMovement mv;
     MsStepExtras ex;
 };
+struct RenderConstsOrder : RenderConsts {
+    int* schedule;
+};
 enum { OUT_INDICES = 1, OUT_LOCATIONS = 2, OUT_DOTS = 4, OUT_DISTANCES = 8, OUT_SCREEN = 16, OUT_RGB = 32, OUT_DEPTH = 64, OUT_CENTRE = 128,
        OUT_SEEN = 256 };
 __global__ __launch_bounds__(WG) void arithmetic_test_kernel(const float* __restrict__ n, const float* __restrict__ d, float* __restrict__ q_inrange,
@@ -96,15 +99,22 @@
     if (r_ieee) r_ieee[i] = sqrtf(x[i]);
 }
 
+__host__ __device__ inline int render_slot(const int b, const int n_blocks) {
+    const int xcd = b & 7, ix = b >> 3;
+    const int q8 = n_blocks >> 3, r8 = n_blocks & 7;
+    return xcd*q8 + (xcd < r8 ? xcd : r8) + ix;
+}
+__host__ __device__ inline void render_fan(const int fan, const int A, const int R, const RenderConsts& rc, int& n, int& a, int& r0, int& span) {
+    const int G = (R + WAVE - 1)/WAVE, F = A*G;
+    n = div_by(fan, rc.by_f); const int rem = fan - n*F; a = div_by(rem, rc.by_g); r0 = (rem - a*G)*WAVE; span = WAVE;
+}
 __host__ __device__ inline bool render_block(const int b, const int n_blocks, const int A, const int R, const int ng, const RenderConsts& rc,
                                              int& n, int& a, int& r0, int& span, int& fan) {
     const int xcd = b & 7, ix = b >> 3;
     fan = b;
     if (ng == 1) {
-        const int q8 = n_blocks >> 3, r8 = n_blocks & 7;
-        fan = xcd*q8 + (xcd < r8 ? xcd : r8) + ix;
-        const int G = (R + WAVE - 1)/WAVE, F = A*G;
-        n = div_by(fan, rc.by_f); const int rem = fan - n*F; a = div_by(rem, rc.by_g); r0 = (rem - a*G)*WAVE; span = WAVE;
+        fan = render_slot(b, n_blocks);
+        render_fan(fan, A, R, rc, n, a, r0, span);
         return true;
     }
     const int NR = ng*WAVE;
@@ -125,7 +135,7 @@
     return true;
 }
 
-__global__ __launch_bounds__(WG) void render_prep_kernel(const MsAgents ag, int* __restrict__ workspace,
+__global__ __launch_bounds__(WG) void render_prep_kernel(const AgentsK ag, int* __restrict__ workspace,
                                                          const int n_agents_total, const int headings_at) {
     const int i = blockIdx.x*WG + threadIdx.x;
     if (i == 0) { workspace[0] = 0; workspace[1] = 0; workspace[2] = 0; workspace[3] = 0; workspace[4] = 0; }
@@ -137,9 +147,10 @@
 }
 
 
-struct RenderArgs { MsScenery sc; MsAgents ag; MsRender out; float agent_radius, half_screen; int R, n_fans; RenderConsts rc; };
+struct RenderArgs { MsScenery sc; AgentsK ag; MsRender out; float agent_radius, half_screen; int R, n_fans; RenderConsts rc; };
 static_assert(offsetof(RenderArgs, ag) == sizeof(MsScenery) && offsetof(RenderArgs, n_fans) + 4 == offsetof(RenderArgs, rc),
               "RenderArgs must mirror render_kernel's parameters");
+struct RenderArgsOrder { MsScenery sc; AgentsK ag; MsRender out; float agent_radius, half_screen; int R, n_fans; RenderConstsOrder rc; };
 typedef const RenderArgs __attribute__((address_space(4)))* LateArgs;
 __device__ inline LateArgs late_args() {
     LateArgs p = (LateArgs)__builtin_amdgcn_kernarg_segment_ptr();
@@ -234,10 +245,11 @@
 #endif
 template <int OBS, int SHADE = 1, int NG = 1, int STEP = 0>
 __global__ __launch_bounds__(WAVE) __attribute__((amdgpu_waves_per_eu(NG > 1 ? MS_WAVES_WIDE : MS_WAVES, NG > 1 ? MS_WAVES_WIDE : MS_WAVES))) void render_kernel(
-        const MsScenery sc, const MsAgents ag, const MsRender out,
+        const MsScenery sc, const AgentsK ag, const MsRender out,
         const float agent_radius, const float half_screen, const int R, const int n_fans,
-        const std::conditional_t<STEP == 1, RenderConstsStep, RenderConsts> rc) {
+        const std::conditional_t<STEP == 1, RenderConstsStep, std::conditional_t<NG == 1, RenderConstsOrder, RenderConsts>> rc) {
     static_assert(STEP == 0 || NG == 1, "the fused step: one group of rays");
+    constexpr bool ORDERED = NG == 1 && STEP == 0;
     PROBE_INIT
     static_assert(NG == 1 || NG == 2 || NG == 4, "one, two or four ray groups per wave");
     [[maybe_unused]] constexpr int NR = WAVE*NG;
@@ -255,7 +267,13 @@
     [[maybe_unused]] int fan = b;
     const int A = sc.n_agents, AF = sc.n_agents*sc.n_model;
     int n, a, r0, span;
-    if (!render_block(b, n_fans, A, R, NG, rc, n, a, r0, span, fan)) return;
+    if constexpr (ORDERED) {
+        const int slot = render_slot(b, n_fans);
+        const int* const at = rc.schedule ? rc.schedule + n_fans + slot : sc.lines_starts;
+        const int named = *at;
+        fan = rc.schedule ? (int)min((unsigned)named, (unsigned)(n_fans - 1)) : slot;
+        render_fan(fan, A, R, rc, n, a, r0, span);
+    } else if (!render_block(b, n_fans, A, R, NG, rc, n, a, r0, span, fan)) return;
     const int r = r0 + lane;
     const int r_last = min(r0 + span - 1, R - 1);
     [[maybe_unused]] const int n_live = r_last - r0 + 1;
@@ -461,6 +479,7 @@
     constexpr bool MASKED = !COLOUR || (OBS >= 1 && NG == 1);
     [[maybe_unused]] const int out_mask_ = MASKED ? (out.obs_subsample >> 8) : 0;
 #define MS_WANTED(BIT, PTR) (MASKED ? ((out_mask_ & (BIT)) != 0) : ((PTR) != nullptr))
+    [[maybe_unused]] int fan_cost = 0;
     auto winner_of = [&](const int nearest_idx, float4& hw_mem, int& tex_w, int& tstart) {
         const LateArgs late = late_args();
         const bool want_texel_row = COLOUR || (OBS && MS_WANTED(OUT_SEEN, late->out.seen_stamp));
@@ -542,9 +561,11 @@
                     reinterpret_cast<LightPair*>(&s_raw[O_EPI]), reinterpret_cast<unsigned*>(&s_raw[O_EPI + 2048]), light_telemetry);
 #endif
                 PROBE_VAL(2, light_telemetry)
+                if constexpr (ORDERED) fan_cost += (light_telemetry & 0x7fu) ? 7 : 0;
             } else if constexpr (NG == 1) {
                 if (out.workspace && lane == 0) out.workspace[16 + atomicAdd(&out.workspace[0], 1)] = fan;
             }
+            if constexpr (ORDERED) fan_cost += 10;
         }
         PROBE_AT(5, tex_w)
         f = tex_filter(is_hit ? loc : 0.f, tex_w);
@@ -553,6 +574,10 @@
         const float* __restrict__ tr = l_tex_vals + 3*(size_t)(tstart + f.r);
         tl0 = tl[0]; tl1 = tl[1]; tl2 = tl[2]; tr0 = tr[0]; tr1 = tr[1]; tr2 = tr[2];
         if (is_hit & !dynamic) intensity = f.lw*bk_l + f.rw*bk_r;
+    }
+    if constexpr (ORDERED) {
+        int* const schedule = reinterpret_cast<const RenderArgsOrder __attribute__((address_space(4)))*>(late)->rc.schedule;
+        if (schedule && lane == 0) schedule[n*A + a] = fan_cost;
     }
     if constexpr (OBS >= 1) {
         if (MS_WANTED(OUT_SEEN, late->out.seen_stamp)) {
@@ -868,6 +893,7 @@
             }
         }
         const unsigned long long amb = __ballot(ambiguous);
+        if constexpr (ORDERED) fan_cost = n_windows + (list_n >> 5) + 4*(int)__popcll(amb);
         PROBE_VAL(11, n_pairs_total) PROBE_VAL(12, n_drains == 1 ? list_n : -1) PROBE_VAL(13, __popcll(amb))
 #if MS_PROBE
         const unsigned t_fold0 = (unsigned)clock64();
@@ -1205,7 +1231,7 @@
 
 
 __global__ __launch_bounds__(WG) void dynlight_kernel(
-        const MsScenery sc, const MsAgents ag, const MsRender out, const int R) {
+        const MsScenery sc, const AgentsK ag, const MsRender out, const int R) {
     __shared__ LightPair s_pair[WAVES][PAIRS];
     __shared__ unsigned s_shadow[2*WAVE];
 
diff --git a/megastep_amd/csrc/megastep_hip.hip b/megastep_amd/csrc/megastep_hip.hip
--- a/megastep_amd/csrc/megastep_hip.hip
+++ b/megastep_amd/csrc/megastep_hip.hip
@@ -24,6 +24,10 @@
 thread_local int g_last_step_fused = 0;
 thread_local int g_last_render_groups = 0;
 thread_local int g_overhead_cull = 1;
+thread_local int g_render_order = 1;
+
+struct AgentsK { float* angles; float* positions; float* angvelocity; float* velocity; float* headings; };
+AgentsK agents_k(const MsAgents& a) { return AgentsK{a.angles, a.positions, a.angvelocity, a.velocity, a.headings}; }
 
 #ifndef MS_PROBE
 #define MS_PROBE 0
@@ -128,7 +132,10 @@
 bool config_ok(const MsConfig* c) {
     return c && c->res > 0 && c->fps > 0.f && c->agent_radius > 0.f && c->fov > 0.f && c->fov < 180.f;
 }
-MsAgents agents_or_none(const MsAgents* a) { return a ? *a : MsAgents{nullptr, nullptr, nullptr, nullptr, nullptr}; }
+AgentsK agents_or_none(const MsAgents* a) { return a ? agents_k(*a) : AgentsK{nullptr, nullptr, nullptr, nullptr, nullptr}; }
+bool schedule_serves(const MsAgents* a, const MsScenery* sc, const int R) {
+    return g_render_order && a->schedule && R <= WAVE && (long long)sc->n_envs*sc->n_agents <= 0x3fffffffLL;
+}
 
 float half_screen_of(const float fov) { return tanf(3.14159265358979323846f/180.f*fov/2.); }
 
@@ -214,6 +221,19 @@
 }
 int ms_debug_ray_group_tail(float rounds, int envs) { g_tail_rounds = rounds; g_tail_envs = envs; return MS_OK; }
 int ms_debug_pair_telemetry(int on) { g_pair_telemetry = on ? 1 : 0; return MS_OK; }
+int ms_debug_render_order(int on) { g_render_order = on ? 1 : 0; return MS_OK; }
+int ms_host_order_fans(int n_fans, const int* costs, int* order) {
+    if (n_fans < 1 || !costs || !order) return -1;
+    const int K = fan_sort_per_run(n_fans);
+    for (int block = 0; block < 8*K; block++) {
+        int first_fan, count, first_slot, next[FAN_CLASSES] = {0};
+        fan_sort_part(n_fans, K, block, first_fan, count, first_slot);
+        for (int i = 0; i < count; i++) next[fan_class(costs[first_fan + i])]++;
+        for (int c = FAN_CLASSES - 1, rank = 0; c >= 0; c--) { const int m = next[c]; next[c] = rank; rank += m; }
+        for (int i = 0; i < count; i++) order[first_slot + K*next[fan_class(costs[first_fan + i])]++] = first_fan + i;
+    }
+    return 8*K;
+}
 
 int ms_test_arithmetic(const float* n, const float* d, float* q_inrange, float* q_ieee, const float* x, float* r_any, float* r_ieee,
                        long long count, void* stream) {
@@ -374,7 +394,7 @@
 int ms_step_physics(const MsScenery* sc, const MsAgents* ag, const MsMovement* mv, const MsStepExtras* ex, float* progress,
                     const MsConfig* cfg, void* stream) {
     if (!scenery_ok(sc) || !agents_ok(ag) || !progress || !config_ok(cfg)) return MS_EINVAL;
-    if (!step_options_ok(mv, ex)) return MS_EINVAL;
+    if (!step_options_ok(mv, ex) || ((uintptr_t)ag->schedule % 4)) return MS_EINVAL;
     if (sc->wg_cells && (!sc->wg_starts || !sc->wg_geom || !sc->wg_near_rows || !(sc->wg_cell > 0.f) || ((uintptr_t)sc->wg_cells % 16) ||
                          ((uintptr_t)sc->wg_geom % 16) || ((uintptr_t)sc->wg_near_rows % 16))) return MS_EINVAL;
     const int pack = physics_pack_of(sc->n_envs, sc->n_agents, sc->wg_cells != nullptr, g_physics_pack);
@@ -386,8 +406,14 @@
     if (!sc->wg_cells) { scn.wg_geom = sc->lines_vals; scn.wg_starts = sc->lines_starts; }
     const hipStream_t hs = (hipStream_t)stream;
     const Divisor by_a = divisor_of((unsigned)sc->n_agents);
+    const AgentsK agk = agents_k(*ag);
+    FanSort fs{nullptr, 0, 1, 0};
+    if (schedule_serves(ag, sc, cfg->res)) {
+        fs.schedule = ag->schedule; fs.n_fans = sc->n_envs*sc->n_agents;
+        fs.per_run = fan_sort_per_run(fs.n_fans); fs.n_blocks = 8*fs.per_run;
+    }
 #define MS_LAUNCH_PHYSICS_P(M, E, P) \
-    hipLaunchKernelGGL((physics_kernel<M, E, P>), dim3((sc->n_envs + pack - 1)/pack), dim3(WAVE), slice*16, hs, scn, *ag, progress, cfg->agent_radius, cfg->fps, mvv, exv, pack, by_a)
+    hipLaunchKernelGGL((physics_kernel<M, E, P>), dim3(fs.n_blocks + (sc->n_envs + pack - 1)/pack), dim3(WAVE), slice*16, hs, scn, agk, progress, cfg->agent_radius, cfg->fps, mvv, exv, pack, by_a, fs)
 #define MS_LAUNCH_PHYSICS(M, E) { if (pack > 1) MS_LAUNCH_PHYSICS_P(M, E, 1); else MS_LAUNCH_PHYSICS_P(M, E, 0); }
     if (mv && ex) MS_LAUNCH_PHYSICS(1, 1)
     else if (ex) MS_LAUNCH_PHYSICS(0, 1)
@@ -410,7 +436,8 @@
 struct RenderLaunch {
     RenderPlan plan;
     RenderConstsStep rc;
-    MsScenery scn; MsAgents agn; MsRender outn;
+    int* schedule;
+    MsScenery scn; AgentsK agn; MsRender outn;
     const MsAgents* ag; const MsRender* out;
     float agent_radius, half_screen; int R;
     bool colour, obs, no_planes;
@@ -464,8 +491,10 @@
     const bool cached = ag->headings && !L.dynlight;
     L.prep = !cached && !L.fused && out->workspace;
     if ((cached && (uintptr_t)ag->headings % 16) || (L.prep && (uintptr_t)out->workspace % 8)) return MS_EINVAL;
-    L.agn = *ag;
+    L.agn = agents_k(*ag);
     L.outn = *out;
+    L.schedule = (schedule_serves(ag, sc, R) && L.plan.ng == 1 && !L.fused) ? ag->schedule : nullptr;
+    if (L.schedule && (uintptr_t)L.schedule % 4) return MS_EINVAL;
     if (!cached && !L.fused) L.agn.headings = nullptr;
     if (!L.prep) L.outn.workspace = nullptr;
     if (out->obs_depth) L.outn.obs_max_depth = 1.f/out->obs_max_depth;
@@ -490,7 +519,9 @@
 static int render_enqueue(const RenderLaunch& L, const hipStream_t hs) {
     g_last_render_groups = L.plan.ng;
     const int na = L.scn.n_envs*L.scn.n_agents;
-    if (L.prep) hipLaunchKernelGGL(render_prep_kernel, dim3((na + WG - 1)/WG), dim3(WG), 0, hs, *L.ag, L.out->workspace, na, L.rc.ws_headings);
+    if (L.prep) hipLaunchKernelGGL(render_prep_kernel, dim3((na + WG - 1)/WG), dim3(WG), 0, hs, agents_k(*L.ag), L.out->workspace, na, L.rc.ws_headings);
+    RenderConstsOrder rco;
+    static_cast<RenderConsts&>(rco) = L.rc; rco.schedule = L.schedule;
 #define MS_LAUNCH_RENDER(O, S, NG_, STEP_) hipLaunchKernelGGL((render_kernel<O, S, NG_, STEP_>), dim3((int)L.plan.n_blocks), dim3(WAVE), 0, hs, \
                                                               L.scn, L.agn, L.outn, L.agent_radius, L.half_screen, L.R, (int)L.plan.n_blocks, L.rc)
 #define MS_LAUNCH_RENDER_OS(NG_) { if (!L.colour) MS_LAUNCH_RENDER(1, 0, NG_, 0); else if (L.no_planes) MS_LAUNCH_RENDER(2, 1, NG_, 0); \
@@ -498,10 +529,16 @@
     if (L.fused) { if (!L.colour) MS_LAUNCH_RENDER(1, 0, 1, 1); else if (L.obs) MS_LAUNCH_RENDER(1, 1, 1, 1); else MS_LAUNCH_RENDER(0, 1, 1, 1); }
     else if (L.plan.ng == 4) MS_LAUNCH_RENDER_OS(4)
     else if (L.plan.ng == 2) MS_LAUNCH_RENDER_OS(2)
-    else MS_LAUNCH_RENDER_OS(1)
+    else {
+#define MS_LAUNCH_RENDER_1(O, S) hipLaunchKernelGGL((render_kernel<O, S, 1, 0>), dim3((int)L.plan.n_blocks), dim3(WAVE), 0, hs, \
+                                                    L.scn, L.agn, L.outn, L.agent_radius, L.half_screen, L.R, (int)L.plan.n_blocks, rco)
+        if (!L.colour) MS_LAUNCH_RENDER_1(1, 0); else if (L.no_planes) MS_LAUNCH_RENDER_1(2, 1);
+        else if (L.obs) MS_LAUNCH_RENDER_1(1, 1); else MS_LAUNCH_RENDER_1(0, 1);
+#undef MS_LAUNCH_RENDER_1
+    }
 #undef MS_LAUNCH_RENDER_OS
 #undef MS_LAUNCH_RENDER
-    if (L.dynlight) hipLaunchKernelGGL(dynlight_kernel, dim3((int)L.plan.n_blocks), dim3(WG), 0, hs, L.scn, *L.ag, *L.out, L.R);
+    if (L.dynlight) hipLaunchKernelGGL(dynlight_kernel, dim3((int)L.plan.n_blocks), dim3(WG), 0, hs, L.scn, agents_k(*L.ag), *L.out, L.R);
     return launch_status();
 }
 
diff --git a/megastep_amd/cuda.py b/megastep_amd/cuda.py
--- a/megastep_amd/cuda.py
+++ b/megastep_amd/cuda.py
@@ -22,6 +22,9 @@
     k = os.environ.get('MEGASTEP_PHYSICS_PACK')
     if k:
         _lib.lib().ms_debug_physics_pack(int(k))
+    o = os.environ.get('MEGASTEP_RENDER_ORDER')
+    if o:
+        _lib.lib().ms_debug_render_order(int(o))
     t, e = os.environ.get('MEGASTEP_RAY_GROUP_TAIL'), os.environ.get('MEGASTEP_RAY_GROUP_TAIL_ENVS')
     if t or e:
         _lib.lib().ms_debug_ray_group_tail(float(t) if t else -1., int(e) if e else -1)
@@ -146,6 +149,7 @@
 class Agents:
 
     HEADING_CACHE = True
+    SCHEDULE = True
 
     def __init__(self, angles, positions, angvelocity, velocity, config=None):
         self._config = config
@@ -157,9 +161,12 @@
         if positions.shape != (n, a, 2) or velocity.shape != (n, a, 2) or angvelocity.shape != (n, a):
             raise RuntimeError('agent tensors must be (N, A), (N, A, 2), (N, A), (N, A, 2)')
         self._headings = torch.full((n, a, 4), float('nan'), dtype=torch.float32, device=angles.device)
+        self._schedule = torch.stack([torch.zeros(n*a, dtype=torch.int32, device=angles.device),
+                                      torch.arange(n*a, dtype=torch.int32, device=angles.device)]) if self.SCHEDULE else None
         ptrs = (angles.data_ptr(), positions.data_ptr(), angvelocity.data_ptr(), velocity.data_ptr())
-        self._struct = _lib.MsAgents(*ptrs, self._headings.data_ptr())
-        self._plain = _lib.MsAgents(*ptrs, None)
+        schedule = self._schedule.data_ptr() if self.SCHEDULE and angles.device.type == 'cuda' else None
+        self._struct = _lib.MsAgents(*ptrs, self._headings.data_ptr(), schedule)
+        self._plain = _lib.MsAgents(*ptrs, None, schedule)
         self._cached = False
         self._epoch = 0
         self._use_cache = bool(self.HEADING_CACHE)
```

After: 105.8 million (median of 6 runs). 7.0% higher.
